# banyancomputer/hot-proofs-blake3-circom

Measured on AMD Instinct MI355X. Metric: BLAKE3-compression witnesses/sec, higher is better.
Workload: dtype u32

## Files before the change

hot-proofs-blake3-circom_amd/build.py:

```python
import os, shutil, subprocess, sys

PKG = os.path.dirname(os.path.abspath(__file__))
ROOT = os.path.dirname(PKG)
CSRC = os.path.join(PKG, "csrc")
LIB = os.path.join(PKG, "libb3wit.so")
NAPI = os.path.join(PKG, "js", "b3wit_napi.node")
ARCH = "gfx950"


def _newer(target, sources):
    if not os.path.exists(target):
        return True
    t = os.path.getmtime(target)
    return any(os.path.getmtime(s) > t for s in sources)


def _run(cmd, **kw):
    print("+", " ".join(cmd), flush=True)
    subprocess.check_call(cmd, **kw)


def hipcc():
    for c in (os.environ.get("HIPCC"), shutil.which("hipcc"), "/opt/rocm/bin/hipcc"):
        if c and os.path.exists(c):
            return c
    raise RuntimeError("hipcc not found")


def build_lib(force=False, extra_flags=()):
    from concurrent.futures import ThreadPoolExecutor
    names = ("b3w_kernels.hip", "b3w_exact.hip", "b3w_plan.hip", "b3w_bao.hip", "b3w_bao_have.hip", "b3w_bao_host.cpp", "b3w_placement.hip", "b3w_commit.hip", "b3w_r1cs.hip", "b3w_r1cs_walk.hip", "b3w_r1cs_host.cpp", "b3w_hostcomm.cpp",
             "b3w_ctx.cpp", "b3w_bodies.cpp", "b3w_wtns.cpp", "b3w_r1cs_api.cpp", "b3w_commit_api.cpp", "b3w_comm.cpp", "b3w_chain.cpp")
    srcs = [os.path.join(CSRC, f) for f in names]
    hdrs = [os.path.join(CSRC, f) for f in sorted(os.listdir(CSRC)) if f.endswith((".h", ".inc"))] + \
        [os.path.join(ROOT, "include", "b3wit.h")]
    objdir = os.path.join(PKG, "build")
    os.makedirs(objdir, exist_ok=True)
    if os.environ.get("B3W_BUILD_DIAG") == "1":
        extra_flags = (*extra_flags, "-DB3W_R1CS_DIAG")
    flags = [f"--offload-arch={ARCH}", "-O3", "-std=c++17", "-fPIC", "-x", "hip", "-Wall", "-Wno-unused-function", *extra_flags]
    jobs = []
    for src in srcs:
        obj = os.path.join(objdir, os.path.basename(src) + ".o")
        if force or extra_flags or _newer(obj, [src] + hdrs):
            jobs.append([hipcc(), *flags, "-c", src, "-o", obj])
    if jobs:
        with ThreadPoolExecutor(max_workers=min(len(jobs), os.cpu_count() or 1)) as ex:
            list(ex.map(_run, jobs))
    objs = [os.path.join(objdir, os.path.basename(src) + ".o") for src in srcs]
    if jobs or _newer(LIB, objs):
        _run([hipcc(), f"--offload-arch={ARCH}", "-fPIC", "-shared", "-o", LIB, *objs, "-ldl", "-lrt", "-lpthread"])
    return LIB


def build_oracle(force=False):
    so = os.path.join(ROOT, "oracle", "libb3w_oracle.so")
    if force or _newer(so, [os.path.join(ROOT, "oracle", "b3w_oracle.c")]):
        _run(["make", "-C", os.path.join(ROOT, "oracle")])
    return so


def build_napi(force=False):
    src = os.path.join(PKG, "js", "b3wit_napi.cc")
    if not os.path.exists(src):
        return None
    inc = "/usr/include/node"
    if not os.path.exists(os.path.join(inc, "node_api.h")):
        print("node_api.h not found; skipping N-API addon", file=sys.stderr)
        return None
    if force or _newer(NAPI, [src, os.path.join(ROOT, "include", "b3wit.h")]):
        _run(["g++", "-O2", "-std=c++17", "-fPIC", "-shared", "-DNODE_GYP_MODULE_NAME=b3wit_napi", "-I", inc,
              "-I", os.path.join(ROOT, "include"), "-o", NAPI, src, "-ldl"])
    return NAPI


def build_all(force=False):
    build_lib(force)
    build_oracle(force)
    build_napi(force)


if __name__ == "__main__":
    build_all(force="--force" in sys.argv)
```

hot-proofs-blake3-circom_amd/csrc/b3w_ctx.cpp:

```cpp
#include "b3w_internal.h"
#include "b3w_layout_tables.inc"
#include "b3w_trace_tables.inc"

namespace {

struct Sha256 {
  uint32_t h[8];
  uint8_t buf[64];
  uint64_t len = 0;
  size_t fill = 0;
  Sha256() {
    static const uint32_t init[8] = {0x6a09e667, 0xbb67ae85, 0x3c6ef372, 0xa54ff53a, 0x510e527f, 0x9b05688c, 0x1f83d9ab, 0x5be0cd19};
    memcpy(h, init, sizeof h);
  }
  static uint32_t ror(uint32_t x, int r) { return (x >> r) | (x << (32 - r)); }
  void block(const uint8_t *p) {
    static const uint32_t K[64] = {
        0x428a2f98, 0x71374491, 0xb5c0fbcf, 0xe9b5dba5, 0x3956c25b, 0x59f111f1, 0x923f82a4, 0xab1c5ed5, 0xd807aa98, 0x12835b01,
        0x243185be, 0x550c7dc3, 0x72be5d74, 0x80deb1fe, 0x9bdc06a7, 0xc19bf174, 0xe49b69c1, 0xefbe4786, 0x0fc19dc6, 0x240ca1cc,
        0x2de92c6f, 0x4a7484aa, 0x5cb0a9dc, 0x76f988da, 0x983e5152, 0xa831c66d, 0xb00327c8, 0xbf597fc7, 0xc6e00bf3, 0xd5a79147,
        0x06ca6351, 0x14292967, 0x27b70a85, 0x2e1b2138, 0x4d2c6dfc, 0x53380d13, 0x650a7354, 0x766a0abb, 0x81c2c92e, 0x92722c85,
        0xa2bfe8a1, 0xa81a664b, 0xc24b8b70, 0xc76c51a3, 0xd192e819, 0xd6990624, 0xf40e3585, 0x106aa070, 0x19a4c116, 0x1e376c08,
        0x2748774c, 0x34b0bcb5, 0x391c0cb3, 0x4ed8aa4a, 0x5b9cca4f, 0x682e6ff3, 0x748f82ee, 0x78a5636f, 0x84c87814, 0x8cc70208,
        0x90befffa, 0xa4506ceb, 0xbef9a3f7, 0xc67178f2};
    uint32_t w[64];
    for (int i = 0; i < 16; i++) w[i] = (uint32_t)p[4 * i] << 24 | (uint32_t)p[4 * i + 1] << 16 | (uint32_t)p[4 * i + 2] << 8 | p[4 * i + 3];
    for (int i = 16; i < 64; i++) {
      uint32_t s0 = ror(w[i - 15], 7) ^ ror(w[i - 15], 18) ^ (w[i - 15] >> 3);
      uint32_t s1 = ror(w[i - 2], 17) ^ ror(w[i - 2], 19) ^ (w[i - 2] >> 10);
      w[i] = w[i - 16] + s0 + w[i - 7] + s1;
    }
    uint32_t a = h[0], b = h[1], c = h[2], d = h[3], e = h[4], f = h[5], g = h[6], hh = h[7];
    for (int i = 0; i < 64; i++) {
      uint32_t t1 = hh + (ror(e, 6) ^ ror(e, 11) ^ ror(e, 25)) + ((e & f) ^ (~e & g)) + K[i] + w[i];
      uint32_t t2 = (ror(a, 2) ^ ror(a, 13) ^ ror(a, 22)) + ((a & b) ^ (a & c) ^ (b & c));
      hh = g; g = f; f = e; e = d + t1; d = c; c = b; b = a; a = t1 + t2;
    }
    h[0] += a; h[1] += b; h[2] += c; h[3] += d; h[4] += e; h[5] += f; h[6] += g; h[7] += hh;
  }
  void update(const uint8_t *p, size_t n) {
    len += n;
    while (n) {
      size_t k = 64 - fill < n ? 64 - fill : n;
      memcpy(buf + fill, p, k);
      fill += k; p += k; n -= k;
      if (fill == 64) { block(buf); fill = 0; }
    }
  }
  void final(uint8_t out[32]) {
    uint64_t bits = len * 8;
    uint8_t pad = 0x80;
    update(&pad, 1);
    uint8_t z = 0;
    while (fill != 56) update(&z, 1);
    uint8_t lb[8];
    for (int i = 0; i < 8; i++) lb[i] = (uint8_t)(bits >> (56 - 8 * i));
    update(lb, 8);
    for (int i = 0; i < 8; i++) { out[4 * i] = h[i] >> 24; out[4 * i + 1] = h[i] >> 16; out[4 * i + 2] = h[i] >> 8; out[4 * i + 3] = h[i]; }
  }
};

const char *const WASM_SHA256[4] = {
    "6faf23ddfd697bbb7e8e922577589c2c06486258968a5a14f96fb5a16091b142",
    "020bd11f289864c54c7d02cd05723dcf8323e31fa5c77d8700c618232685978e",
    "b982f960ebbfcabe957fe13857ea47adfeee30e18fbe05474e9b982eab187f46",
    "8d6317b72eab34d34e12dfd7bd310dce40f4190768669772f992a9510c441fca"};


uint64_t fnv1a64(const char *s) {
  uint64_t h = 0xCBF29CE484222325ull;
  for (; *s; ++s) { h ^= (uint8_t)*s; h *= 0x100000001B3ull; }
  return h;
}
const CircuitDesc CIRCUITS[4] = {
    {B3W_KIND_COMP, 24093, 28, 16, P_BN254, B3W_LAYOUT_0, B3W_LAYOUT_0_NRUNS, B3W_LDS_WORDS_COMP},
    {B3W_KIND_NOVA_O2, 23291, 32, 15, P_BN254, B3W_LAYOUT_1, B3W_LAYOUT_1_NRUNS, B3W_LDS_WORDS_NOVA_O2},
    {B3W_KIND_NOVA_O2, 23291, 32, 15, P_VESTA, B3W_LAYOUT_2, B3W_LAYOUT_2_NRUNS, B3W_LDS_WORDS_NOVA_O2},
    {B3W_KIND_NOVA_O1, 24614, 32, 15, P_BN254, B3W_LAYOUT_3, B3W_LAYOUT_3_NRUNS, B3W_LDS_WORDS_NOVA_O1},
};

bool atom_lds(int kind, uint32_t atom, uint32_t *word, int *width ) {
  if (atom < B3W_A_HG) { *word = atom; *width = 32; return true; }
  if (atom < B3W_A_NV) {
    const uint32_t k = (atom - B3W_A_HG) / 8, j = (atom - B3W_A_HG) % 8;
    static const uint32_t off[8] = {0, 0, 2, 2, 4, 5, 6, 7};
    *word = B3W_LDS_HG + 8 * k + off[j];
    *width = (j == B3W_HG_S1 || j == B3W_HG_S3) ? 64 : 32;
    return true;
  }
  if (kind == B3W_KIND_COMP) return false;
  const uint32_t i = atom - B3W_A_NV;
  if (i == NV_CHUNK_IDX) { *word = B3W_LDS_CHUNK_IDX; *width = 64; return true; }
  if (i < NV_NARROW_COUNT) { *word = B3W_LDS_NV + i; *width = 32; return true; }
  if (i >= NV_COUNT) return false;
  uint32_t j = i - NV_NARROW_COUNT;
  if (kind == B3W_KIND_NOVA_O2) {
    if (j < 3) {  }
    else if (i >= NV_EQ_INV && i < NV_EQ_INV + 64) j = 3 + (i - NV_EQ_INV);
    else return false;
  }
  *word = B3W_LDS_WIDE + 8 * j;
  *width = 256;
  return true;
}

void inv_small_host(uint32_t k, const uint32_t P[8], uint32_t out[8]) {
  uint64_t r = 0;
  for (int i = 7; i >= 0; --i) r = ((r << 32) | P[i]) % k;
  int64_t x0 = 0, x1 = 1;
  uint64_t a = k, b = r;
  while (b > 1) {
    const uint64_t q = a / b, tt = a - q * b;
    a = b; b = tt;
    const int64_t tx = x0 - (int64_t)q * x1;
    x0 = x1; x1 = tx;
  }
  int64_t x = x1 % (int64_t)k;
  if (x < 0) x += k;
  const uint64_t t = ((uint64_t)k - (uint64_t)x) % k;
  uint32_t prod[9];
  uint64_t carry = 1;
  for (int i = 0; i < 8; ++i) {
    const uint64_t cur = (uint64_t)P[i] * t + carry;
    prod[i] = (uint32_t)cur;
    carry = cur >> 32;
  }
  prod[8] = (uint32_t)carry;
  uint64_t rem = 0;
  for (int i = 8; i >= 0; --i) {
    const uint64_t cur = (rem << 32) | prod[i];
    const uint64_t qd = cur / k;
    rem = cur - qd * k;
    if (i < 8) out[i] = (uint32_t)qd;
  }
}
std::vector<uint32_t> build_nova_aux(const uint64_t *prime) {
  std::vector<uint32_t> aux(16 + 8 * B3W_INV_TABLE_N, 0);
  memcpy(aux.data(), prime, 32);
  aux[8] = B3W_INV_TABLE_N;
  for (uint32_t k = 1; k < B3W_INV_TABLE_N; ++k) inv_small_host(k, aux.data(), aux.data() + 16 + 8 * k);
  return aux;
}

bool build_slot_table(const CircuitDesc &c, std::vector<uint32_t> &table, std::string &err) {
  const uint32_t padded = ((c.nwit + 31) / 32 + 8) * 32;
  table.assign(padded, B3W_ENTRY(0, 31, B3W_MODE_BIT));
  std::vector<uint8_t> seen(c.nwit, 0);
  char msg[128];
  for (uint32_t r = 0; r < c.nruns; r++) {
    const b3w_layout_run &run = c.runs[r];
    for (uint32_t j = 0; j < run.len; j++) {
      const uint32_t slot = run.slot + j;
      if (slot >= c.nwit || seen[slot]) { err = "layout: bad or duplicate slot"; return false; }
      seen[slot] = 1;
      uint32_t word; int width;
      if (run.kind == 'W') {
        if (!atom_lds(c.kind, run.atom + j, &word, &width)) {
          snprintf(msg, sizeof msg, "layout: atom %u not staged for this circuit kind", run.atom + j);
          err = msg; return false;
        }
        table[slot] = B3W_ENTRY(word, 0, width == 32 ? B3W_MODE_W32 : width == 64 ? B3W_MODE_W64 : B3W_MODE_W256);
      } else {
        const uint32_t bit = run.bit0 + j;
        if (run.atom == B3W_A_NV + NV_CHUNK_IDX && bit == 64) {
          table[slot] = B3W_ENTRY(B3W_A_ONE, 31, B3W_MODE_BIT);
          continue;
        }
        if (!atom_lds(c.kind, run.atom, &word, &width) || (int)bit >= width || width == 256) {
          snprintf(msg, sizeof msg, "layout: bit %u of atom %u not expressible", bit, run.atom);
          err = msg; return false;
        }
        table[slot] = B3W_ENTRY(word + bit / 32, bit % 32, B3W_MODE_BIT);
      }
    }
  }
  for (uint32_t s = 0; s < c.nwit; s++) if (!seen[s]) { err = "layout: uncovered slot"; return false; }
  return true;
}

bool build_exact_table(const CircuitDesc &c, std::vector<uint32_t> &table) {
  table.assign(c.nwit, 0);
  for (uint32_t r = 0; r < c.nruns; r++) {
    const b3w_layout_run &run = c.runs[r];
    for (uint32_t j = 0; j < run.len; j++) {
      const uint32_t slot = run.slot + j;
      if (slot >= c.nwit) return false;
      if (run.kind == 'W') table[slot] = (run.atom + j) | (0xFFFFu << 16);
      else table[slot] = (run.atom == B3W_A_NV + NV_CIL ? B3W_A_NV + NV_CHUNK_IDX : run.atom) | ((run.bit0 + j) << 16);
    }
  }
  return true;
}

bool reference_trace(int circuit, uint32_t site, std::string &text) {
  static const b3w_trace_entry *const T[4] = {B3W_TRACES_0, B3W_TRACES_1, B3W_TRACES_2, B3W_TRACES_3};
  static const uint32_t N[4] = {B3W_TRACES_0_N, B3W_TRACES_1_N, B3W_TRACES_2_N, B3W_TRACES_3_N};
  const uint32_t code = site & 0xFF, r = (site >> 8) & 0xF;
  const bool later = code == 1 && r >= 1 && r <= 6;
  const uint32_t key = later ? site & ~0xF00u : site;
  for (uint32_t i = 0; i < N[circuit]; i++) {
    if (T[circuit][i].site != key) continue;
    text = T[circuit][i].text;
    if (!later) return true;
    const std::string frame = "Error in template Blake3Compression_";
    const size_t at = text.find(frame), num = at == std::string::npos ? at : text.find(" line: ", at), end = num == std::string::npos ? num : text.find('\n', num);
    if (end == std::string::npos) return false;
    text.replace(num + 7, end - (num + 7), circuit == 0 ? "207" : "208");
    return true;
  }
  return false;
}

bool build_input_slots(const CircuitDesc &c, std::vector<uint32_t> &slots) {
  slots.assign(c.nin, 0xFFFFFFFFu);
  const uint32_t first = c.kind == B3W_KIND_COMP ? B3W_A_H : B3W_A_NV;
  for (uint32_t r = 0; r < c.nruns; r++) {
    const b3w_layout_run &run = c.runs[r];
    if (run.kind != 'W') continue;
    for (uint32_t j = 0; j < run.len; j++) {
      const uint32_t atom = run.atom + j;
      if (atom >= first && atom < first + c.nin && slots[atom - first] == 0xFFFFFFFFu) slots[atom - first] = run.slot + j;
    }
  }
  for (uint32_t v : slots) if (v == 0xFFFFFFFFu) return false;
  return true;
}

const char *assert_site_text(uint32_t site, char *buf, size_t len) {
  const uint32_t code = site & 0xFF, r = (site >> 8) & 0xF, g = (site >> 12) & 0xF, hf = (site >> 16) & 1;
  switch (code) {
    case 1: snprintf(buf, len, "Error in template Bits34 line: 201 (rounds[%u].GS[%u].half%u.add1)\n", r, g, hf + 1); break;
    case 2: snprintf(buf, len, "Error in template ToBits line: 153 (rounds[%u].GS[%u].half%u.rxor2.tb)\n", r, g, hf + 1); break;
    case 3: snprintf(buf, len, "Error in template Bits33 line: 176 (rounds[%u].GS[%u].half%u.add3)\n", r, g, hf + 1); break;
    case 4: snprintf(buf, len, "Error in template ToBits line: 153 (rounds[%u].GS[%u].half%u.rxor4.tb)\n", r, g, hf + 1); break;
    case 5: snprintf(buf, len, "Error in template ToBits line: 153 (outXor[%u].tb_x)\n", g + 8 * hf); break;
    case 6: snprintf(buf, len, "Error in template ToBits line: 153 (outXor[%u].tb_y)\n", g + 8 * hf); break;
    case 10: snprintf(buf, len, "Error in template Num2Bits line: 38 (check_depth.check_parent.n2b)\n"); break;
    case 11: snprintf(buf, len, "Error in template Num2Bits line: 38 (check_depth.exceed_depth.lt.n2b)\n"); break;
    case 12: snprintf(buf, len, "Error in template Blake3NovaTreePath_CheckDepth line: 38\n"); break;
    case 13: snprintf(buf, len, "Error in template Num2Bits line: 38 (final_m.down_left_path.n2b)\n"); break;
    case 14: snprintf(buf, len, "Error in template Blake3GetDownLeftPath line: 77\n"); break;
    default: snprintf(buf, len, "assert site %u\n", site);
  }
  return buf;
}

}

bool b3w_int_build_slot_table(const CircuitDesc &c, std::vector<uint32_t> &table, std::string &err) { return build_slot_table(c, table, err); }

namespace {
int32_t ensure_scratch(b3w_ctx *ctx) {
  if (ctx->d_scratch) return B3W_OK;
  ctx->scratch_cap = B3W_SWEEP_CHUNK;
  hipError_t e = hipMalloc((void **)&ctx->d_scratch, (size_t)ctx->scratch_cap * ctx->desc.lds_words * 4);
  if (e != hipSuccess) { ctx->scratch_cap = 0; return hip_fail(ctx, e, "hipMalloc(sweep scratch)"); }
  return B3W_OK;
}

void set_inputs(b3w_ctx *ctx) {
  struct Def { const char *name; uint32_t count; };
  static const Def comp[] = {{"h", 8}, {"m", 16}, {"t", 2}, {"b", 1}, {"d", 1}};
  static const Def nova[] = {{"n_blocks", 1}, {"block_count", 1}, {"h", 8}, {"chunk_idx_low", 1}, {"chunk_idx_high", 1},
                             {"leaf_depth", 1}, {"total_depth", 1}, {"depth", 1}, {"m", 16}, {"b", 1}};
  const Def *d = ctx->desc.kind == B3W_KIND_COMP ? comp : nova;
  const int nd = ctx->desc.kind == B3W_KIND_COMP ? 5 : 10;
  uint32_t off = 0;
  for (int i = 0; i < nd; i++) {
    ctx->inputs.push_back({d[i].name, d[i].count, off, fnv1a64(d[i].name)});
    off += d[i].count;
  }
}
}

int b3w_int_default_variant(const b3w_ctx *ctx, uint32_t n, const uint8_t *d_bodies, uint64_t pitch) {
  const bool comp = ctx->desc.kind == B3W_KIND_COMP, nova2 = ctx->desc.kind == B3W_KIND_NOVA_O2;
  const bool fillable = ctx->fill_ok && !(reinterpret_cast<uintptr_t>(d_bodies) & 31) && !(pitch & 31) && pitch < (1ull << 30) &&
                        (uint64_t)n * pitch + (1ull << 20) < (1ull << 37);
  if (fillable && comp && n >= 128 && (n <= 3072 || !b3w_place_is_mixed(d_bodies))) return B3W_VARIANT_REGIONFILL;
  if (fillable && nova2 && (b3w_place_is_mixed(d_bodies) ? n >= 768 && n <= 2560 : n >= 512)) return B3W_VARIANT_REGIONFILL;
  if (n <= 2560) return B3W_VARIANT_SLICED + (n <= (comp ? 32u : 8u) ? 64 : n <= 96 ? 32 : n <= 192 ? 16 : n <= 768 ? 8 : 4);
  if (comp) return n <= 6144 ? 0 : 8;
  if (nova2) return n <= 3072 ? 0 : n <= 32768 ? 3 : 4;
  return 0;
}

extern "C" {

uint32_t b3w_abi_version(void) { return (1u << 16) | 4u; }

int32_t b3w_identify_wasm(const uint8_t *code, size_t len) {
  if (!code) return B3W_CIRCUIT_UNKNOWN;
  Sha256 s;
  s.update(code, len);
  uint8_t dg[32];
  s.final(dg);
  char hex[65];
  for (int i = 0; i < 32; i++) snprintf(hex + 2 * i, 3, "%02x", dg[i]);
  for (int c = 0; c < 4; c++) if (!strcmp(hex, WASM_SHA256[c])) return c;
  return B3W_CIRCUIT_UNKNOWN;
}

int32_t b3w_create(int32_t circuit, int32_t device, b3w_ctx **out) {
  if (!out || circuit < 0 || circuit > 3) return B3W_E_BAD_ARGUMENT;
  *out = nullptr;
  int ndev = 0;
  if (hipGetDeviceCount(&ndev) != hipSuccess || ndev <= 0 || device < 0 || device >= ndev) return B3W_E_NO_DEVICE;
  b3w_ctx *ctx = new b3w_ctx;
  ctx->circuit = circuit;
  ctx->desc = CIRCUITS[circuit];
  ctx->device = device;
  set_inputs(ctx);
  std::vector<uint32_t> table;
  if (!build_slot_table(ctx->desc, table, ctx->last_error)) { delete ctx; return B3W_E_BAD_ARGUMENT; }
  std::vector<uint32_t> wide_slots(B3W_NOVA_ISZERO, 0xFFFFFFFFu);
  ctx->fill_ok = ctx->desc.kind == B3W_KIND_COMP || ctx->desc.kind == B3W_KIND_NOVA_O2;
  for (uint32_t i = 0; i < table.size(); i++) {
    const uint32_t e = table[i], src = e & 0xFFFu, sh = (e >> 12) & 31u, mode = (e >> 17) & 3u;
    if (mode != B3W_MODE_BIT && sh != 0) ctx->fill_ok = false;
    if (ctx->desc.kind == B3W_KIND_COMP) {
      if (src >= 1023 || mode == B3W_MODE_W256) ctx->fill_ok = false;
    } else if (mode == B3W_MODE_W256) {
      const uint32_t j = src >= B3W_LDS_WIDE && (src - B3W_LDS_WIDE) % 8 == 0 ? (src - B3W_LDS_WIDE) / 8 : 0xFFFFFFFFu;
      if (j >= B3W_NOVA_ISZERO || wide_slots[j] != 0xFFFFFFFFu) ctx->fill_ok = false; else wide_slots[j] = i;
    } else if (src + (mode == B3W_MODE_W64 ? 1u : 0u) >= B3W_LDS_WIDE) ctx->fill_ok = false;
  }
  if (ctx->desc.kind == B3W_KIND_NOVA_O2) {
    for (uint32_t v : wide_slots) if (v == 0xFFFFFFFFu) ctx->fill_ok = false;
    for (uint32_t j = 0; ctx->fill_ok && j < B3W_NOVA_ISZERO; j++) {
      if (j > 0 && wide_slots[j] <= wide_slots[j - 1]) ctx->fill_ok = false;
      for (int d = -3; ctx->fill_ok && d <= 3; d++) {
        const int64_t k = (int64_t)wide_slots[j] + d;
        if (k < 0 || k >= (int64_t)ctx->desc.nwit) continue;
        const uint32_t e = table[k], src = e & 0xFFFu, mode = (e >> 17) & 3u;
        if (mode != B3W_MODE_W256 && !((src >= B3W_A_H && src < B3W_A_O) || src >= B3W_LDS_NV)) ctx->fill_ok = false;
      }
    }
  }
  std::vector<uint16_t> ftab(table.size(), 0);
  std::vector<uint32_t> alias;
  if (ctx->fill_ok) {
    const bool nova = ctx->desc.kind != B3W_KIND_COMP;
    std::vector<uint8_t> used(4097, 0);
    for (uint32_t i = 0; i < ctx->desc.nwit; i++) {
      const uint32_t e = table[i], src = e & 0xFFFu, mode = (e >> 17) & 3u;
      if (mode == B3W_MODE_W256) continue;
      used[src] = 1;
      if (mode == B3W_MODE_W64) used[src + 1] = 1;
    }
    used[B3W_LDS_OKWORD] = used[B3W_LDS_OKWORD + 1] = 1;
    for (uint32_t k = 0; k < 16; k++) used[B3W_A_O + k] = 1;
    if (nova) for (uint32_t k : {NV_N_BLOCKS, NV_BLOCK_COUNT_OUT, NV_TOTAL_DEPTH, NV_DEPTH_OUT, NV_CIL, NV_CIH, NV_LEAF_DEPTH}) used[B3W_LDS_NV + k] = 1;
    for (uint32_t w = 2048; w < 4097; w++) if (used[w]) ctx->fill_ok = false;
    std::vector<uint16_t> to(2048, 0xFFFFu);
    uint32_t hole = B3W_LDS_HG;
    for (uint32_t w = 1024; w < 2048 && ctx->fill_ok; w++) {
      if (!used[w]) continue;
      while (hole < 1024 && used[hole]) hole++;
      if (hole >= 1024 || alias.size() >= B3W_ALIAS_MAX) { ctx->fill_ok = false; break; }
      used[hole] = 1; to[w] = (uint16_t)hole;
      alias.push_back(w | hole << 16);
    }
    for (uint32_t i = 0; i < table.size() && ctx->fill_ok; i++) {
      const uint32_t e = table[i], sh = (e >> 12) & 31u, mode = (e >> 17) & 3u;
      uint32_t src = e & 0xFFFu;
      if (mode == B3W_MODE_W256) { ftab[i] = (uint16_t)(0x8000u | 2u << 10); continue; }
      if (src >= 1024) {
        if (mode == B3W_MODE_W64 || src >= 2048 || to[src] == 0xFFFFu) { if (i < ctx->desc.nwit) ctx->fill_ok = false; continue; }
        src = to[src];
      }
      if (mode == B3W_MODE_W64 && src + 1 >= 1024) { ctx->fill_ok = false; continue; }
      ftab[i] = (uint16_t)(mode == B3W_MODE_BIT ? (src | sh << 10) : (src | (mode == B3W_MODE_W64 ? 1u : 0u) << 10 | 0x8000u));
    }
  }
  DeviceGuard guard(device);
  if (guard.err != hipSuccess) { delete ctx; return B3W_E_NO_DEVICE; }
  const CircuitDesc &d = ctx->desc;
  hipError_t e = hipMalloc((void **)&ctx->d_table_base, (table.size() + 32) * 4 + ftab.size() * 2);
  if (e == hipSuccess) e = hipMemset(ctx->d_table_base, 0, 32 * 4);
  if (e == hipSuccess) ctx->d_table = ctx->d_table_base + 32;
  if (e == hipSuccess) e = hipMemcpy(ctx->d_table, table.data(), table.size() * 4, hipMemcpyHostToDevice);
  if (e == hipSuccess) e = hipMemcpy(ctx->d_table + table.size(), ftab.data(), ftab.size() * 2, hipMemcpyHostToDevice);
  if (e == hipSuccess && d.kind != B3W_KIND_COMP) {
    std::vector<uint32_t> aux = build_nova_aux(d.prime);
    static_assert(B3W_AUX_WIDE_SLOTS == 16 + 8 * B3W_INV_TABLE_N, "b3w_kernels.h and b3w_internal.h disagree about the inverse table");
    aux.insert(aux.end(), wide_slots.begin(), wide_slots.end());
    if (ctx->fill_ok && d.kind == B3W_KIND_NOVA_O2) {
      aux.resize(B3W_AUX_LINE_LISTS + 2 * 4 * B3W_LINE_LIST_MAX, 0xFFFFFFFFu);
      for (uint32_t ph = 0; ph < 4; ph++) {
        uint32_t cnt = 0, last_line = 0xFFFFFFFFu;
        for (uint32_t j = 0; j < B3W_NOVA_ISZERO; j++) {
          const uint32_t line = (ph + wide_slots[j]) >> 2;
          if (line == last_line) continue;
          last_line = line;
          for (uint32_t i = 0; i < 4; i++) {
            const uint32_t k = line * 4 + i - ph;
            if (k >= d.nwit) continue;
            if (cnt == B3W_LINE_LIST_MAX) { ctx->fill_ok = false; break; }
            aux[B3W_AUX_LINE_LISTS + 2 * (ph * B3W_LINE_LIST_MAX + cnt)] = k;
            aux[B3W_AUX_LINE_LISTS + 2 * (ph * B3W_LINE_LIST_MAX + cnt) + 1] = table[k];
            cnt++;
          }
        }
        aux[B3W_AUX_LINE_COUNTS + ph] = cnt;
      }
      aux.resize(B3W_AUX_ALIAS_LIST + B3W_ALIAS_MAX, 0u);
      aux[B3W_AUX_ALIAS_COUNT] = (uint32_t)alias.size();
      for (size_t k = 0; k < alias.size(); k++) aux[B3W_AUX_ALIAS_LIST + k] = alias[k];
    }
    e = hipMalloc(&ctx->d_aux, aux.size() * 4);
    if (e == hipSuccess) e = hipMemcpy(ctx->d_aux, aux.data(), aux.size() * 4, hipMemcpyHostToDevice);
  }
  {
    std::vector<uint32_t> xt;
    if (!build_exact_table(d, xt)) { b3w_destroy(ctx); return B3W_E_BAD_ARGUMENT; }
    if (e == hipSuccess) e = hipMalloc((void **)&ctx->d_exact_table, xt.size() * 4);
    if (e == hipSuccess) e = hipMemcpy(ctx->d_exact_table, xt.data(), xt.size() * 4, hipMemcpyHostToDevice);
    if (e == hipSuccess) e = hipMalloc((void **)&ctx->d_prime, 32);
    if (e == hipSuccess) e = hipMemcpy(ctx->d_prime, d.prime, 32, hipMemcpyHostToDevice);
    if (e == hipSuccess) e = hipMalloc((void **)&ctx->d_fe_inputs, 32 * 32);
    if (e == hipSuccess) e = hipMalloc((void **)&ctx->d_status2, 8);
    std::vector<uint32_t> ins;
    if (build_input_slots(d, ins)) {
      if (e == hipSuccess) e = hipMalloc((void **)&ctx->d_in_slots, ins.size() * 4);
      if (e == hipSuccess) e = hipMemcpy(ctx->d_in_slots, ins.data(), ins.size() * 4, hipMemcpyHostToDevice);
    }
  }
  if (e == hipSuccess) e = hipMalloc((void **)&ctx->d_rec1, d.nin * 4);
  if (e == hipSuccess) e = hipMalloc((void **)&ctx->d_body1, (size_t)d.nwit * 32);
  if (e == hipSuccess) e = hipMalloc((void **)&ctx->d_status1, 4);
  if (e != hipSuccess) { b3w_destroy(ctx); return B3W_E_HIP; }
  const char *v = getenv("B3W_VARIANT");
  if (v) { ctx->variant = atoi(v); ctx->variant_auto = false; }
  if (ctx->variant >= B3W_VARIANT_SWEEP && ctx->variant < B3W_VARIANT_REGIONFILL && ensure_scratch(ctx) != B3W_OK) { b3w_destroy(ctx); return B3W_E_HIP; }
  *out = ctx;
  return B3W_OK;
}

void b3w_destroy(b3w_ctx *ctx) {
  if (!ctx) return;
  B3wCaptureRelaxed relaxed;
  DeviceGuard guard(ctx->device);
  (void)b3w_ctx_trim(ctx);
  if (ctx->d_table_base) (void)hipFree(ctx->d_table_base);
  if (ctx->d_aux) (void)hipFree(ctx->d_aux);
  if (ctx->d_scratch) (void)hipFree(ctx->d_scratch);
  if (ctx->d_exact_table) (void)hipFree(ctx->d_exact_table);
  if (ctx->d_prime) (void)hipFree(ctx->d_prime);
  if (ctx->d_fe_inputs) (void)hipFree(ctx->d_fe_inputs);
  if (ctx->d_status2) (void)hipFree(ctx->d_status2);
  if (ctx->d_in_slots) (void)hipFree(ctx->d_in_slots);
  if (ctx->d_rec1) (void)hipFree(ctx->d_rec1);
  if (ctx->d_body1) (void)hipFree(ctx->d_body1);
  if (ctx->d_status1) (void)hipFree(ctx->d_status1);
  if (ctx->samples_done) { (void)hipEventSynchronize(ctx->samples_done); (void)hipEventDestroy(ctx->samples_done); }
  if (ctx->h_samples) (void)hipHostFree(ctx->h_samples);
  if (ctx->d_samples) (void)hipFree(ctx->d_samples);
  if (ctx->batch_done) { (void)hipEventSynchronize(ctx->batch_done); (void)hipEventDestroy(ctx->batch_done); }
  if (ctx->h_batch) (void)hipHostFree(ctx->h_batch);
  if (ctx->d_batch) (void)hipFree(ctx->d_batch);
  for (b3w_ctx::ManySlot &m : ctx->many_slots) {
    if (m.done) { if (m.busy) (void)hipEventSynchronize(m.done); (void)hipEventDestroy(m.done); }
    if (m.h) (void)hipHostFree(m.h);
    if (m.d) (void)hipFree(m.d);
  }
  delete ctx;
}

int32_t b3w_info(const b3w_ctx *ctx, uint32_t *n32, uint8_t prime_le[32], uint32_t *witness_size,
                 uint32_t *input_size, uint32_t version[3]) {
  if (!ctx) return B3W_E_BAD_ARGUMENT;
  if (n32) *n32 = 8;
  if (prime_le) memcpy(prime_le, ctx->desc.prime, 32);
  if (witness_size) *witness_size = ctx->desc.nwit;
  if (input_size) *input_size = ctx->desc.nin;
  if (version) { version[0] = 2; version[1] = 1; version[2] = 6; }
  return B3W_OK;
}

int32_t b3w_input_signal_size(const b3w_ctx *ctx, uint64_t h) {
  if (!ctx) return 0;
  for (const InputSignal &s : ctx->inputs) if (s.hash == h) return (int32_t)s.count;
  return 0;
}

uint32_t b3w_public_words(const b3w_ctx *ctx) { return ctx ? ctx->desc.npub : 0; }

int32_t b3w_last_error(const b3w_ctx *ctx, char *buf, size_t len) {
  if (!ctx || !buf || !len) return B3W_E_BAD_ARGUMENT;
  snprintf(buf, len, "%s", ctx->last_error.c_str());
  return B3W_OK;
}

int32_t b3w_write_wtns_header(const b3w_ctx *ctx, uint8_t out[76]) {
  if (!ctx || !out) return B3W_E_BAD_ARGUMENT;
  uint32_t w[19];
  memcpy(&w[0], "wtns", 4);
  w[1] = 2; w[2] = 2;
  w[3] = 1; w[4] = 8 + 32; w[5] = 0;
  w[6] = 32;
  memcpy(&w[7], ctx->desc.prime, 32);
  w[15] = ctx->desc.nwit;
  const uint64_t len = 32ull * ctx->desc.nwit;
  w[16] = 2; w[17] = (uint32_t)len; w[18] = (uint32_t)(len >> 32);
  memcpy(out, w, 76);
  return B3W_OK;
}

int32_t b3w_batch_run_device(b3w_ctx *ctx, const uint32_t *d_records, uint32_t n, uint8_t *d_bodies, uint64_t pitch,
                             uint32_t *d_public, int32_t *d_status, void *stream) {
  if (!ctx || !d_records || !d_bodies) return B3W_E_BAD_ARGUMENT;
  const uint64_t body = 32ull * ctx->desc.nwit;
  if (pitch == 0) pitch = body;
  if (pitch < body || (pitch & 31)) { ctx->last_error = "pitch must be >= witness_size*32 and a multiple of 32"; return B3W_E_BAD_ARGUMENT; }
  if (reinterpret_cast<uintptr_t>(d_bodies) & 15) { ctx->last_error = "d_bodies must be 16-byte aligned"; return B3W_E_BAD_ARGUMENT; }
  ON_DEVICE(ctx);
  int variant = ctx->variant;
  if (ctx->variant_auto || (ctx->variant_tuned && n <= 2560)) variant = b3w_int_default_variant(ctx, n, d_bodies, pitch);
  if (variant >= B3W_VARIANT_REGIONFILL && !ctx->fill_ok) { ctx->last_error = "the fill-ordered variants (200, 201) exist for the compression circuit and the nova O2 builds"; return B3W_E_BAD_ARGUMENT; }
  int rc = b3w_launch_batch(ctx->desc.kind, variant, d_records, n, d_bodies, pitch, ctx->d_table, ctx->desc.nwit,
                            d_public, d_status, ctx->d_aux, ctx->d_scratch, ctx->scratch_cap, (hipStream_t)stream);
  if (rc == 0) return B3W_OK;
  if (rc == -5) { ctx->last_error = "the sweep and fill-ordered paths need 32-byte aligned bodies and pitch < 2^30"; return B3W_E_BAD_ARGUMENT; }
  if (rc < 0) { ctx->last_error = "no kernel for this circuit kind / variant"; return B3W_E_BAD_ARGUMENT; }
  return hip_fail(ctx, (hipError_t)rc, "kernel launch");
}

int32_t b3w_batch_verify_device(b3w_ctx *ctx, const uint8_t *d_bodies, uint32_t n, uint64_t pitch, uint32_t *d_mismatch,
                                void *stream) {
  if (!ctx || !d_bodies || !d_mismatch) return B3W_E_BAD_ARGUMENT;
  if (!ctx->d_in_slots) { ctx->last_error = "this circuit's layout does not keep every input as a slot"; return B3W_E_BAD_ARGUMENT; }
  const uint64_t body = 32ull * ctx->desc.nwit;
  if (pitch == 0) pitch = body;
  if (pitch < body || (pitch & 31) || (reinterpret_cast<uintptr_t>(d_bodies) & 15)) {
    ctx->last_error = "pitch must be >= witness_size*32 and a multiple of 32, bodies 16-byte aligned";
    return B3W_E_BAD_ARGUMENT;
  }
  ON_DEVICE(ctx);
  int rc = b3w_launch_verify(ctx->desc.kind, ctx->d_in_slots, n, d_bodies, pitch, ctx->d_table, ctx->desc.nwit, d_mismatch,
                             ctx->d_aux, (hipStream_t)stream);
  return rc ? hip_fail(ctx, (hipError_t)rc, "verify launch") : B3W_OK;
}

int32_t b3w_batch_autotune_device(b3w_ctx *ctx, const uint32_t *d_records, uint32_t n, uint8_t *d_bodies, uint64_t pitch,
                                  uint32_t *d_public, int32_t *d_status, void *stream, int32_t *chosen_variant,
                                  float *chosen_ms) {
  if (!ctx || !d_records || !d_bodies || !n) return B3W_E_BAD_ARGUMENT;
  ON_DEVICE(ctx);
  int32_t rc;
  if (n <= 2560 && (ctx->variant_auto || ctx->variant_tuned)) {
    float ms = 0;
    rc = B3W_OK;
    for (int w = 0; w < 2 && rc == B3W_OK; w++) rc = b3w_batch_run_device(ctx, d_records, n, d_bodies, pitch, d_public, d_status, stream);
    if (rc == B3W_OK) rc = b3w_batch_time_device(ctx, d_records, n, d_bodies, pitch, d_public, d_status, stream, 5, &ms);
    if (rc) return rc;
    if (chosen_variant) *chosen_variant = b3w_int_default_variant(ctx, n, d_bodies, pitch ? pitch : 32ull * ctx->desc.nwit);
    if (chosen_ms) *chosen_ms = ms;
    return B3W_OK;
  }
  rc = ensure_scratch(ctx);
  if (rc) return rc;
  const int candidates[6] = {0, ctx->desc.kind == B3W_KIND_COMP ? (n > 6144 ? 8 : 3) : ctx->desc.kind == B3W_KIND_NOVA_O2 ? 3 : 0, B3W_VARIANT_SWEEP,
                             ctx->fill_ok ? B3W_VARIANT_REGIONFILL : 0, ctx->desc.kind == B3W_KIND_NOVA_O2 && n >= 16384 ? 4 : 0,
                             ctx->fill_ok ? B3W_VARIANT_REGIONFILL_LIGHT : 0};
  int best = ctx->variant;
  float best_ms = 1e30f;
  const int saved = ctx->variant;
  const bool saved_auto = ctx->variant_auto;
  ctx->variant_auto = false;
  float cand_ms[6] = {1e30f, 1e30f, 1e30f, 1e30f, 1e30f, 1e30f};
  for (int round = 0; round < 2; round++) {
    for (int ci = 0; ci < 6; ci++) {
      const int c = candidates[ci];
      if (ci > 0 && c == candidates[0]) continue;
      if (round > 0 && cand_ms[ci] >= 1e30f) continue;
      ctx->variant = c;
      float ms = 0;
      rc = B3W_OK;
      for (int w = 0; w < 2 && rc == B3W_OK; w++)
        rc = b3w_batch_run_device(ctx, d_records, n, d_bodies, pitch, d_public, d_status, stream);
      if (rc == B3W_OK) rc = b3w_batch_time_device(ctx, d_records, n, d_bodies, pitch, d_public, d_status, stream, n <= 8192 ? 20 : 5, &ms);
      if (rc == B3W_E_BAD_ARGUMENT) continue;
      if (rc) { ctx->variant = saved; ctx->variant_auto = saved_auto; return rc; }
      if (ms < cand_ms[ci]) cand_ms[ci] = ms;
    }
  }
  for (int ci = 0; ci < 6; ci++)
    if (cand_ms[ci] < best_ms) { best_ms = cand_ms[ci]; best = candidates[ci]; }
  if (best_ms >= 1e30f) { ctx->variant = saved; ctx->variant_auto = saved_auto; return B3W_E_BAD_ARGUMENT; }
  ctx->variant = best;
  ctx->variant_tuned = true;
  if (chosen_variant) *chosen_variant = best;
  if (chosen_ms) *chosen_ms = best_ms;
  return B3W_OK;
}

int32_t b3w_batch_time_device(b3w_ctx *ctx, const uint32_t *d_records, uint32_t n, uint8_t *d_bodies, uint64_t pitch,
                              uint32_t *d_public, int32_t *d_status, void *stream, uint32_t iters, float *avg_ms) {
  if (!ctx || !avg_ms || !iters) return B3W_E_BAD_ARGUMENT;
  ON_DEVICE(ctx);
  hipEvent_t e0 = nullptr, e1 = nullptr;
  hipError_t e = hipEventCreate(&e0);
  if (e == hipSuccess) e = hipEventCreate(&e1);
  if (e == hipSuccess) e = hipEventRecord(e0, (hipStream_t)stream);
  int32_t rc = B3W_OK;
  for (uint32_t i = 0; i < iters && e == hipSuccess && rc == B3W_OK; i++)
    rc = b3w_batch_run_device(ctx, d_records, n, d_bodies, pitch, d_public, d_status, stream);
  float ms = 0;
  if (e == hipSuccess && rc == B3W_OK) e = hipEventRecord(e1, (hipStream_t)stream);
  if (e == hipSuccess && rc == B3W_OK) e = hipEventSynchronize(e1);
  if (e == hipSuccess && rc == B3W_OK) e = hipEventElapsedTime(&ms, e0, e1);
  if (e0) (void)hipEventDestroy(e0);
  if (e1) (void)hipEventDestroy(e1);
  if (rc) return rc;
  if (e != hipSuccess) return hip_fail(ctx, e, "timing events");
  *avg_ms = ms / iters;
  return B3W_OK;
}

static int32_t calc_witness_run(b3w_ctx *ctx, const std::vector<uint32_t> &rec, const std::vector<uint8_t> &fe, bool canonical,
                                uint8_t *out_body) {
  const CircuitDesc &d = ctx->desc;
  char msg[200];
  ON_DEVICE(ctx);
  if (canonical) {
    HIP_TRY(ctx, hipMemcpy(ctx->d_rec1, rec.data(), d.nin * 4, hipMemcpyHostToDevice));
    int32_t rc = b3w_batch_run_device(ctx, ctx->d_rec1, 1, ctx->d_body1, 0, nullptr, ctx->d_status1, nullptr);
    if (rc) return rc;
    int32_t st = 0;
    HIP_TRY(ctx, hipMemcpy(&st, ctx->d_status1, 4, hipMemcpyDeviceToHost));
    if (st == 0) {
      HIP_TRY(ctx, hipMemcpy(out_body, ctx->d_body1, (size_t)d.nwit * 32, hipMemcpyDeviceToHost));
      return B3W_OK;
    }
  }
  HIP_TRY(ctx, hipMemcpy(ctx->d_fe_inputs, fe.data(), fe.size(), hipMemcpyHostToDevice));
  int rc = b3w_launch_exact(d.kind != B3W_KIND_COMP, ctx->d_fe_inputs, ctx->d_prime, ctx->d_exact_table, d.nwit,
                            ctx->d_body1, ctx->d_status2, nullptr);
  if (rc) return hip_fail(ctx, (hipError_t)rc, "exact kernel launch");
  uint32_t st2[2] = {0, 0};
  HIP_TRY(ctx, hipMemcpy(st2, ctx->d_status2, 8, hipMemcpyDeviceToHost));
  if (st2[0] != 0) {
    if (!reference_trace(ctx->circuit, st2[1], ctx->last_error))
      ctx->last_error = std::string("Assert Failed.\n") + assert_site_text(st2[1], msg, sizeof msg);
    return B3W_E_ASSERT_FAILED;
  }
  HIP_TRY(ctx, hipMemcpy(out_body, ctx->d_body1, (size_t)d.nwit * 32, hipMemcpyDeviceToHost));
  return B3W_OK;
}

int32_t b3w_calc_witness(b3w_ctx *ctx, const uint64_t *name_hashes, const uint32_t *counts, const uint8_t *values_le32,
                         uint32_t nkeys, uint8_t *out_body) {
  if (!ctx || !name_hashes || !counts || !values_le32 || !out_body) return B3W_E_BAD_ARGUMENT;
  const CircuitDesc &d = ctx->desc;
  std::vector<uint32_t> rec(d.nin, 0);
  std::vector<uint8_t> fe((size_t)d.nin * 32, 0);
  std::vector<uint8_t> set(d.nin, 0);
  uint32_t nset = 0;
  bool canonical = true, ran = false;
  const uint8_t *v = values_le32;
  char msg[200];
  for (uint32_t k = 0; k < nkeys; k++) {
    const InputSignal *sig = nullptr;
    for (const InputSignal &s : ctx->inputs) if (s.hash == name_hashes[k]) sig = &s;
    const uint32_t size = sig ? sig->count : 0;
    if (counts[k] < size) { ctx->last_error = std::string("Not enough values for input signal ") + (sig ? sig->name : "?") + "\n"; return B3W_E_ARRAY_ACCESS; }
    if (counts[k] > size) { ctx->last_error = std::string("Too many values for input signal ") + (sig ? sig->name : "?") + "\n"; return B3W_E_TOO_MANY_SIGNALS; }
    for (uint32_t i = 0; i < size; i++, v += 32) {
      const uint32_t idx = sig->rec_off + i;
      if (set[idx]) { ctx->last_error = "Signal already set.\n"; return B3W_E_SIGNAL_ALREADY_SET; }
      memcpy(&fe[(size_t)idx * 32], v, 32);
      memcpy(&rec[idx], v, 4);
      for (int b = 4; b < 32; b++) canonical &= (v[b] == 0);
      set[idx] = 1;
      nset++;
    }
    if (!ran && size > 0 && nset == d.nin) {
      const int32_t rc = calc_witness_run(ctx, rec, fe, canonical, out_body);
      if (rc) return rc;
      ran = true;
    }
  }
  if (nset < d.nin) {
    snprintf(msg, sizeof msg, "Not all inputs have been set. Only %u out of %u", nset, d.nin);
    ctx->last_error = msg;
    return B3W_E_NOT_ALL_INPUTS;
  }
  return B3W_OK;
}

}
```

hot-proofs-blake3-circom_amd/csrc/b3w_internal.h:

```cpp
#pragma once
#include <hip/hip_runtime_api.h>
#include <hip/hip_ext.h>
#include <errno.h>
#include <fcntl.h>
#include <stdint.h>
#include <stdio.h>
#include <stdlib.h>
#include <string.h>
#include <sys/uio.h>
#include <unistd.h>
#include <algorithm>
#include <array>
#include <chrono>
#include <atomic>
#include <map>
#include <mutex>
#include <thread>
#include <string>
#include <vector>

#include "../../include/b3wit.h"
#include "b3w_atoms.h"
#include "b3w_capture.h"
#include "b3w_kernels.h"
#include "b3w_r1cs_host.h"


struct b3w_layout_run { char kind; uint32_t slot, atom, bit0, len; };

struct InputSignal { const char *name; uint32_t count; uint32_t rec_off; uint64_t hash; };

struct CircuitDesc {
  int kind;
  uint32_t nwit, nin, npub;
  const uint64_t *prime;
  const b3w_layout_run *runs;
  uint32_t nruns;
  uint32_t lds_words;
};
inline constexpr uint64_t P_BN254[4] = {0x43e1f593f0000001ull, 0x2833e84879b97091ull, 0xb85045b68181585dull, 0x30644e72e131a029ull};
inline constexpr uint64_t P_VESTA[4] = {0x8c46eb2100000001ull, 0x224698fc0994a8ddull, 0x0ull, 0x4000000000000000ull};
constexpr uint32_t B3W_INV_TABLE_N = 2048;

struct b3w_ctx {
  int circuit = -1;
  CircuitDesc desc{};
  int device = -1;
  int variant = 0;
  bool variant_auto = true;
  bool fill_ok = false;
  bool variant_tuned = false;
  std::vector<InputSignal> inputs;
  uint32_t *d_table = nullptr;
  uint32_t *d_table_base = nullptr;
  void *d_aux = nullptr;
  uint32_t *d_scratch = nullptr;
  uint32_t *d_exact_table = nullptr;
  uint32_t *d_prime = nullptr;
  uint32_t *d_fe_inputs = nullptr;
  uint32_t *d_status2 = nullptr;
  uint32_t *d_in_slots = nullptr;
  uint32_t scratch_cap = 0;
  uint32_t *d_rec1 = nullptr;
  uint8_t *d_body1 = nullptr;
  int32_t *d_status1 = nullptr;
  float plain_ms_per_gb = 0;
  struct Spare { void *ptr; uint64_t bytes; int32_t placement; };
  std::vector<Spare> ring_spares;
  uint64_t *h_samples = nullptr, *d_samples = nullptr;
  uint32_t samples_cap = 0;
  hipEvent_t samples_done = nullptr;
  uint8_t *h_batch = nullptr, *d_batch = nullptr;
  uint64_t batch_cap = 0;
  hipEvent_t batch_done = nullptr;
  static constexpr uint32_t B3W_MANY_SLOTS = 8;
  struct ManySlot { uint8_t *h = nullptr, *d = nullptr; uint64_t cap = 0; hipEvent_t done = nullptr; bool busy = false; };
  ManySlot many_slots[B3W_MANY_SLOTS];
  uint32_t many_next = 0;
  std::string last_error;
};

struct b3w_batch {
  b3w_ctx *ctx = nullptr;
  uint32_t capacity = 0, n = 0;
  uint64_t pitch = 0;
  int32_t placement = B3W_PLACEMENT_PLAIN;
  uint32_t *d_recs = nullptr;
  uint8_t *d_bodies = nullptr;
  uint32_t *d_pub = nullptr;
  int32_t *d_status = nullptr;
};

inline int32_t hip_fail(b3w_ctx *ctx, hipError_t e, const char *what) {
  if (ctx) ctx->last_error = std::string(what) + ": " + hipGetErrorString(e);
  return B3W_E_HIP;
}
inline int32_t refuse(b3w_ctx *ctx, const char *call, const std::string &why) {
  ctx->last_error = call ? std::string(call) + ": " + why : why;
  return B3W_E_BAD_ARGUMENT;
}
inline int32_t group_log_ok(b3w_ctx *ctx, const char *call, uint32_t group_log) {
  return group_log > B3W_BAO_MAX_GROUP_LOG ? refuse(ctx, call, "group_log is above B3W_BAO_MAX_GROUP_LOG (6)") : B3W_OK;
}
#define HIP_TRY(ctx, call)                                  \
  do {                                                      \
    hipError_t _e = (call);                                 \
    if (_e != hipSuccess) return hip_fail(ctx, _e, #call);  \
  } while (0)

#define B3W_TRY(...)                  \
  do {                                \
    const int32_t _rc = (__VA_ARGS__);\
    if (_rc) return _rc;              \
  } while (0)

struct DeviceGuard {
  int prev = -1;
  bool switched = false;
  hipError_t err = hipSuccess;
  explicit DeviceGuard(int dev) {
    err = hipGetDevice(&prev);
    if (err == hipSuccess && prev != dev) {
      err = hipSetDevice(dev);
      switched = err == hipSuccess;
    }
  }
  ~DeviceGuard() { if (switched) (void)hipSetDevice(prev); }
  DeviceGuard(const DeviceGuard &) = delete;
  DeviceGuard &operator=(const DeviceGuard &) = delete;
};
#define ON_DEVICE(ctx)                         \
  DeviceGuard _dev_guard((ctx)->device);       \
  if (_dev_guard.err != hipSuccess) return hip_fail(ctx, _dev_guard.err, "hipSetDevice")

bool b3w_int_build_slot_table(const CircuitDesc &c, std::vector<uint32_t> &table, std::string &err);
int b3w_int_default_variant(const b3w_ctx *ctx, uint32_t n, const uint8_t *d_bodies, uint64_t pitch);
b3w_ctx *b3w_int_key_ctx(const b3w_commit_key *key);
int32_t b3w_int_commit_records(b3w_ctx *ctx, const b3w_commit_key *key, const uint32_t *d_records, uint32_t n, uint8_t *d_points, uint32_t *d_public,
                               int32_t *d_status, void *stream, uint32_t *d_sums_out, void *trace_stream = nullptr, hipEvent_t trace_done = nullptr);
int32_t b3w_int_commit_normalize(b3w_ctx *ctx, const b3w_commit_key *key, const uint32_t *d_sums, uint64_t n, uint8_t *d_points, void *stream);
b3w_ctx *b3w_int_r1cs_ctx(const b3w_r1cs *r1cs);
int32_t b3w_int_batch_staging(b3w_ctx *ctx, uint64_t bytes);
int32_t b3w_int_batch_launched(b3w_ctx *ctx, hipStream_t st, const char *what);
constexpr uint64_t B3W_RING_SPARE_CAP = 26ull << 30;
```

hot-proofs-blake3-circom_amd/csrc/b3w_kernels.h:

```cpp
#pragma once
#include <hip/hip_runtime_api.h>
#include <stdint.h>

#define B3W_VARIANT_SWEEP 100
#define B3W_VARIANT_SLICED 20
#define B3W_VARIANT_REGIONFILL 200
#define B3W_VARIANT_REGIONFILL_LIGHT 201
#define B3W_REGIONFILL_GRID 256
#define B3W_AUX_WIDE_SLOTS (16 + 8 * 2048)
#define B3W_AUX_LINE_COUNTS (B3W_AUX_WIDE_SLOTS + 68)
#define B3W_AUX_LINE_LISTS (B3W_AUX_LINE_COUNTS + 4)
#define B3W_LINE_LIST_MAX 160
#define B3W_AUX_ALIAS_COUNT (B3W_AUX_LINE_LISTS + 2 * 4 * B3W_LINE_LIST_MAX)
#define B3W_AUX_ALIAS_LIST (B3W_AUX_ALIAS_COUNT + 1)
#define B3W_ALIAS_MAX 192
#define B3W_SWEEP_GRID 256
#define B3W_SWEEP_LOGC 13
#define B3W_SWEEP_CHUNK (1u << B3W_SWEEP_LOGC)

extern "C" int b3w_launch_batch(int kind, int variant, const uint32_t *d_recs, uint32_t n, uint8_t *d_out,
                                uint64_t pitch, const uint32_t *d_table, uint32_t nwit, uint32_t *d_pub,
                                int32_t *d_status, const void *d_aux, uint32_t *d_scratch, uint32_t scratch_cap,
                                hipStream_t stream);

extern "C" int b3w_launch_exact(int nova, const uint32_t *d_inputs, const uint32_t *d_prime, const uint32_t *d_table,
                                uint32_t nwit, uint8_t *d_out, uint32_t *d_status, hipStream_t stream);

extern "C" uint32_t b3w_plan_path_len(uint64_t chunk, uint64_t nchunks);
extern "C" int b3w_launch_plan_leaves(const uint8_t *d_pre, uint64_t total_len, uint64_t first_chunk, uint32_t nlocal,
                                      uint64_t nchunks, uint32_t *d_recs, uint32_t *d_chunk_cv, hipStream_t stream);
extern "C" int b3w_launch_plan_merge(const uint32_t *d_left, const uint32_t *d_right, uint32_t stride_words, uint64_t npairs,
                                     uint32_t root, uint32_t *d_parents, hipStream_t stream);
extern "C" int b3w_launch_plan_parents(const uint32_t *d_levels, uint64_t nchunks, uint64_t first_chunk, uint32_t nlocal,
                                       uint32_t last_chunk_blocks, uint32_t *d_recs, hipStream_t stream);
extern "C" uint32_t b3w_plan_tree_first_level(uint64_t nchunks);
extern "C" int b3w_launch_plan_tree(uint32_t *d_levels, uint64_t nchunks, uint32_t l0, uint32_t *d_root, uint64_t first_chunk, uint32_t plan_nlocal,
                                    uint32_t last_chunk_blocks, uint32_t *d_recs, hipStream_t stream);
extern "C" uint64_t b3w_plan_parent_row(uint64_t chunk, uint64_t nchunks);
extern "C" int b3w_plan_path_provable(uint64_t chunk, uint64_t nchunks);
extern "C" int b3w_launch_pack_hout(const uint32_t *d_pub, uint64_t row0, uint64_t count, uint32_t *d_dst, hipStream_t stream);
extern "C" int b3w_launch_unpack_hout(const uint32_t *d_gathered, uint64_t block_words, uint64_t par_off, const uint64_t *d_tab, uint32_t nranks,
                                      uint64_t max_rows, uint32_t *d_leaf_all, uint32_t *d_par_all, hipStream_t stream);

extern "C" int b3w_launch_trace(int kind, const uint32_t *d_recs, uint32_t cn, uint32_t *d_images, uint32_t row, const uint32_t *d_table,
                                uint32_t nwit, uint32_t *d_pub, int32_t *d_status, const void *d_aux, hipStream_t stream);
extern "C" int b3w_launch_verify(int kind, const uint32_t *d_in_slots, uint32_t n, const uint8_t *d_bodies, uint64_t pitch,
                                 const uint32_t *d_table, uint32_t nwit, uint32_t *d_mismatch, const void *d_aux,
                                 hipStream_t stream);

extern "C" int b3w_place_alloc(int device, uint64_t bytes, int want_mixed, void **out, int *mixed, float *rates);
extern "C" int b3w_place_free(void *ptr);
extern "C" int b3w_place_is_mixed(const void *ptr);
extern "C" void b3w_place_trim(void);
extern "C" void b3w_place_configure(int64_t search_gib, int64_t pool_gib);
extern "C" void b3w_place_stats(int device, uint64_t out[6]);
extern "C" void b3w_place_search_limit(double seconds);
extern "C" void b3w_place_search_stats(int device, double out[4]);
extern "C" void b3w_place_cost_breakdown(int device, double out[4]);
extern "C" int b3w_place_store_rate(uint8_t *buf, uint64_t pitch, uint32_t n, uint32_t body_bytes, int shape, uint32_t iters, hipStream_t stream, double *gbs);

#define B3W_COMMIT_WINDOW_SMALL 12
#define B3W_COMMIT_WINDOW_LARGE 16
#define B3W_COMMIT_WINDOW_XL 18
#define B3W_COMMIT_WINDOW_OK(w) ((w) == B3W_COMMIT_WINDOW_SMALL || (w) == B3W_COMMIT_WINDOW_LARGE || (w) == B3W_COMMIT_WINDOW_XL)
#define B3W_COMMIT_ENTRIES(W) ((1u << (W)) - 1u)
#define B3W_COMMIT_SUM_WORDS 36
#include "b3w_commit_curve.h"
extern "C" int b3w_launch_commit_setup(const uint32_t *d_gens, const uint32_t *d_first_v, const uint32_t *d_nbits, uint32_t nslots,
                                       uint32_t *d_points, const B3wCurve *curve, hipStream_t stream);
extern "C" int b3w_launch_commit_windows(const uint32_t *d_points, uint32_t nwin, uint32_t window, uint32_t *d_table, const B3wCurve *curve, hipStream_t stream);
extern "C" int b3w_launch_commit(const uint8_t *d_bodies, uint32_t n, uint64_t pitch, uint32_t first_slot, uint32_t nslots,
                                 const uint32_t *d_slotdesc ,
                                 const uint32_t *d_images ,
                                 uint32_t img_row, const uint32_t *d_runs , uint32_t nruns,
                                 const uint32_t *d_table, uint32_t nwin, uint32_t window, uint32_t *d_sums, uint8_t *d_out,
                                 int32_t *d_status, const uint32_t *d_invtab , uint32_t inv_nk,
                                 const uint32_t *d_invmeta ,
                                 const uint32_t *d_aux ,
                                 unsigned long long *d_adds ,
                                 const B3wCurve *curve, hipStream_t stream);
extern "C" int b3w_launch_commit_normalize(const uint32_t *d_sums, uint64_t n, uint8_t *d_out, const B3wCurve *curve, hipStream_t stream);
#define B3W_NOVA_ISZERO 67
extern "C" int b3w_launch_commit_invtab(const uint32_t *d_gens, const uint32_t *d_inv_slot, const uint32_t *d_inverses, uint32_t njobs, uint32_t nk,
                                        uint32_t *d_invtab, const B3wCurve *curve, hipStream_t stream);

#include "b3w_r1cs_defs.h"
extern "C" int b3w_launch_r1cs(const uint8_t *d_bodies, uint32_t n, uint64_t pitch, uint32_t m, const uint32_t *d_rows,
                               const uint32_t *d_row_id, const uint32_t *d_wires, const uint16_t *d_cids, const uint32_t *d_coefR,
                               const B3wField *field, uint32_t *d_violations, uint32_t *d_first, hipStream_t stream);
struct B3wR1csSystem {
  uint32_t nwires, ntiles, max_ext, max_tile_terms, max_tile_rows, ncoef;
  const uint32_t *tiles, *tile_terms, *ext, *rows, *row_id, *row_k, *terms, *coefs;
  const long long *coef_small;
  const uint32_t *g_rows, *g_wires;
  const uint16_t *g_cids;
  uint32_t max_g_words, max_g_rows, smask_groups;
  const uint32_t *srows, *sgdesc, *sgwords, *sgmeta;
  const unsigned long long *smask;
  const unsigned long long *scost;
};
struct B3wWalk {
  uint32_t ntiles, exp_slots, max_gen, max_ent, ncoef, static_words, max_rows, signed_elems;
  const uint32_t *tile;
  const unsigned long long *mask;
  const uint16_t *exp;
  const uint4 *runs;
  const uint32_t *run_row, *ent_w, *ent_m, *row_id;
  const unsigned long long *stat;
  const long long *coef_small;
  const uint32_t *static_k, *static_id;
  uint32_t nstatic, pad2;
  uint32_t static_d0[4];
  uint32_t p[8];
};
extern "C" int b3w_launch_r1cs_walk(const uint8_t *d_bodies, uint32_t n, uint64_t pitch, const B3wWalk *walk, const B3wR1csSystem *sysw, const B3wField *field,
                                    unsigned long long *d_scratch, uint32_t *d_violations, uint32_t *d_first, hipStream_t stream);
extern "C" size_t b3w_r1cs_walk_scratch_bytes(const B3wWalk *walk);
#define B3W_R1CS_SLAB 8192u
extern "C" size_t b3w_r1cs_scratch_bytes(const B3wR1csSystem *sys);
extern "C" int b3w_launch_r1cs_stream(const uint8_t *d_bodies, uint32_t n, uint64_t pitch, const B3wR1csSystem *sys, const B3wField *field,
                                      unsigned long long *d_scratch, uint32_t *d_violations, uint32_t *d_first, hipStream_t stream);
```

hot-proofs-blake3-circom_amd/csrc/b3w_kernels.hip:

```cpp
#include <hip/hip_runtime.h>
#include <stdint.h>
#include <stdlib.h>
#include <atomic>
#include "b3w_atoms.h"
#include "b3w_kernels.h"

namespace {

typedef uint32_t u32x4 __attribute__((ext_vector_type(4)));

__device__ __forceinline__ uint32_t rotr32(uint32_t x, int r) { return __builtin_rotateright32(x, r); }

template <int P0, int P1, int P2, int P3>
__device__ __forceinline__ uint32_t quad_perm(uint32_t x) {
  return (uint32_t)__builtin_amdgcn_update_dpp(0, (int)x, P0 | (P1 << 2) | (P2 << 4) | (P3 << 6), 0xF, 0xF, false);
}

__host__ __device__ constexpr uint64_t sched_pack(int r) {
  const int sigma[16] = {2, 6, 3, 10, 7, 0, 4, 13, 1, 11, 12, 5, 9, 14, 15, 8};
  int p[16] = {0, 1, 2, 3, 4, 5, 6, 7, 8, 9, 10, 11, 12, 13, 14, 15};
  for (int i = 0; i < r; i++) {
    int q[16] = {};
    for (int j = 0; j < 16; j++) q[j] = p[sigma[j]];
    for (int j = 0; j < 16; j++) p[j] = q[j];
  }
  uint64_t v = 0;
  for (int j = 0; j < 16; j++) v |= (uint64_t)p[j] << (4 * j);
  return v;
}

template <int R1, int R2>
__device__ __forceinline__ void half_g(uint32_t &a, uint32_t &b, uint32_t &c, uint32_t &d, uint32_t m,
                                       uint32_t *Lk) {
  const uint64_t s1 = (uint64_t)a + b + m;
  const uint32_t A = (uint32_t)s1;
  const uint32_t D2 = rotr32(d ^ A, R1);
  const uint64_t s3 = (uint64_t)c + D2;
  const uint32_t C = (uint32_t)s3;
  const uint32_t B4 = rotr32(b ^ C, R2);
  *reinterpret_cast<uint4 *>(Lk) = make_uint4(A, (uint32_t)(s1 >> 32), C, (uint32_t)(s3 >> 32));
  *reinterpret_cast<uint4 *>(Lk + 4) = make_uint4(D2, d, B4, b);
  a = A; d = D2; c = C; b = B4;
}

template <int R>
__device__ __forceinline__ void round_fn(uint32_t &a, uint32_t &b, uint32_t &c, uint32_t &d, const uint32_t *L,
                                         uint32_t *Lw, int col) {
  constexpr uint64_t P = sched_pack(R);
  const uint32_t *M = L + B3W_A_M;
  {
    const uint32_t mx = M[(P >> (8 * col)) & 15], my = M[(P >> (8 * col + 4)) & 15];
    uint32_t *Lk = Lw + B3W_LDS_HG + 8 * ((R * 8 + col) * 2);
    half_g<16, 12>(a, b, c, d, mx, Lk);
    half_g<8, 7>(a, b, c, d, my, Lk + 8);
  }
  b = quad_perm<1, 2, 3, 0>(b);
  c = quad_perm<2, 3, 0, 1>(c);
  d = quad_perm<3, 0, 1, 2>(d);
  {
    const uint32_t mx = M[(P >> (32 + 8 * col)) & 15], my = M[(P >> (36 + 8 * col)) & 15];
    uint32_t *Lk = Lw + B3W_LDS_HG + 8 * ((R * 8 + 4 + col) * 2);
    half_g<16, 12>(a, b, c, d, mx, Lk);
    half_g<8, 7>(a, b, c, d, my, Lk + 8);
  }
  b = quad_perm<3, 0, 1, 2>(b);
  c = quad_perm<2, 3, 0, 1>(c);
  d = quad_perm<1, 2, 3, 0>(d);
}

__device__ __forceinline__ void trace_compression(uint32_t *L, int col, uint32_t *pub ) {
  const uint32_t IVc = col == 0 ? 0x6A09E667u : col == 1 ? 0xBB67AE85u : col == 2 ? 0x3C6EF372u : 0xA54FF53Au;
  uint32_t a = L[B3W_A_H + col], b = L[B3W_A_H + 4 + col], c = IVc, d = L[B3W_A_T + col];
  const uint32_t h_lo = a, h_hi = b;
  round_fn<0>(a, b, c, d, L, L, col);
  round_fn<1>(a, b, c, d, L, L, col);
  round_fn<2>(a, b, c, d, L, L, col);
  round_fn<3>(a, b, c, d, L, L, col);
  round_fn<4>(a, b, c, d, L, L, col);
  round_fn<5>(a, b, c, d, L, L, col);
  round_fn<6>(a, b, c, d, L, L, col);
  const uint32_t o0 = a ^ c, o1 = b ^ d, o2 = c ^ h_lo, o3 = d ^ h_hi;
  L[B3W_A_O + col] = o0;
  L[B3W_A_O + 4 + col] = o1;
  L[B3W_A_O + 8 + col] = o2;
  L[B3W_A_O + 12 + col] = o3;
  if (col == 0) L[B3W_A_ONE] = 1u;
  if (pub) { pub[col] = o0; pub[4 + col] = o1; pub[8 + col] = o2; pub[12 + col] = o3; }
}

template <bool NT>
__device__ __forceinline__ void store16(uint8_t *p, uint4 v) {
  const u32x4 x = {v.x, v.y, v.z, v.w};
  if (NT) __builtin_nontemporal_store(x, reinterpret_cast<u32x4 *>(p));
  else *reinterpret_cast<u32x4 *>(p) = x;
}

template <int W, int WORDS, bool WIDE, bool NT, bool FULL>
__device__ __forceinline__ void emit_group(const uint32_t *lds, uint32_t e, uint8_t *__restrict__ out,
                                           const uint64_t (&woff)[W], uint32_t byte_off, bool in, uint32_t nact,
                                           const uint32_t *okmask) {
  const uint32_t par = threadIdx.x & 1;
  const uint32_t src = e & 0xFFFu, sh = (e >> 12) & 31u, mode = (e >> 17) & 3u;
  const uint32_t off = (WIDE && mode == B3W_MODE_W256) ? src + 4u * par : src;
  const bool live = (par == 0) || (WIDE && mode == B3W_MODE_W256);
  const uint32_t m0 = live ? (mode == B3W_MODE_BIT ? 1u : 0xFFFFFFFFu) : 0u;
  const uint32_t m1 = (live && mode >= B3W_MODE_W64) ? 0xFFFFFFFFu : 0u;
  const uint32_t m23 = (WIDE && mode == B3W_MODE_W256) ? 0xFFFFFFFFu : 0u;
#pragma unroll
  for (int w = 0; w < W; ++w) {
    if (FULL || ((uint32_t)w < nact && (!okmask || okmask[w]))) {
      const uint32_t *L = lds + w * WORDS + off;
      uint4 v;
      v.x = (L[0] >> sh) & m0;
      v.y = L[1] & m1;
      if (WIDE) { v.z = L[2] & m23; v.w = L[3] & m23; } else { v.z = 0; v.w = 0; }
      if (FULL || in) store16<NT>(out + woff[w] + byte_off, v);
    }
  }
}

struct WaveBodies {
  uint32_t first, stride;
  __device__ __forceinline__ uint32_t operator()(int w) const { return first + (uint32_t)w * stride; }
};
template <int W>
__device__ __forceinline__ WaveBodies wave_bodies(uint32_t bid, uint32_t stride) {
  return WaveBodies{(bid / stride) * (stride * W) + bid % stride, stride};
}
template <int W>
__device__ __forceinline__ uint32_t wave_active(const WaveBodies &wb, uint32_t n) {
  uint32_t a = 0;
#pragma unroll
  for (int w = 0; w < W; ++w) a += wb(w) < n ? 1u : 0u;
  return a;
}

template <int W, int WORDS, bool WIDE, bool NT>
__device__ __forceinline__ void expand(const uint32_t *lds, const uint32_t *__restrict__ table, uint32_t nwit,
                                       uint8_t *__restrict__ out, uint64_t pitch, const WaveBodies wb, uint32_t n,
                                       const uint32_t *okmask , bool all_ok,
                                       uint32_t slice = 0, uint32_t slices = 1 ) {
  constexpr int U = 4;
  const int lane = threadIdx.x;
  const uint32_t nact = wave_active<W>(wb, n);
  const uint64_t start = reinterpret_cast<uint64_t>(out) + (uint64_t)wb.first * pitch;
  const uint32_t j = (start & 31) ? 0u : (uint32_t)(start >> 5) & 3u;
  const uint32_t ntiles = (nwit + j + 31) >> 5;
  const uint32_t kf0 = j ? 1u : 0u, kf1 = (nwit + j) >> 5;
  uint64_t woff[W];
#pragma unroll
  for (int w = 0; w < W; ++w) woff[w] = (uint64_t)wb(w) * pitch + (uint32_t)lane * 16u - 32u * j;
  const uint32_t *tp = table + (lane >> 1) - j;
  uint32_t k = 0, kend_all = ntiles;
  if (slices > 1) {
    const uint32_t per = ((ntiles + slices - 1) / slices + (U - 1)) & ~(uint32_t)(U - 1);
    k = slice * per < ntiles ? slice * per : ntiles;
    kend_all = k + per < ntiles ? k + per : ntiles;
#pragma unroll
    for (int w = 0; w < W; ++w) woff[w] += (uint64_t)k * 1024u;
  }
  const uint32_t kf1s = kf1 < kend_all ? kf1 : kend_all;
  auto ragged = [&](uint32_t kend) {
    for (; k < kend; ++k) {
      const uint32_t slot = k * 32 + (lane >> 1) - j;
      emit_group<W, WORDS, WIDE, NT, false>(lds, tp[k * 32], out, woff, 0, slot < nwit, nact, okmask);
#pragma unroll
      for (int w = 0; w < W; ++w) woff[w] += 1024u;
    }
  };
  if (nact == (uint32_t)W && all_ok) {
    ragged(kf0 < kend_all ? kf0 : kend_all);
    uint32_t cur[U], nxt[U];
#pragma unroll
    for (int u = 0; u < U; ++u) cur[u] = tp[(k + u) * 32];
    for (; k + U <= kf1s; k += U) {
#pragma unroll
      for (int u = 0; u < U; ++u) nxt[u] = tp[(k + U + u) * 32];
#pragma unroll
      for (int u = 0; u < U; ++u) emit_group<W, WORDS, WIDE, NT, true>(lds, cur[u], out, woff, u * 1024u, true, nact, nullptr);
#pragma unroll
      for (int w = 0; w < W; ++w) woff[w] += U * 1024u;
#pragma unroll
      for (int u = 0; u < U; ++u) cur[u] = nxt[u];
    }
  }
  ragged(kend_all);
}

template <int W, int WORDS, bool WIDE>
__device__ __forceinline__ void expand_verify(const uint32_t *lds, const uint32_t *__restrict__ table, uint32_t nwit,
                                              const uint8_t *__restrict__ bodies, uint64_t pitch, const WaveBodies wb, uint32_t n,
                                              uint32_t (&cnt)[W]) {
  constexpr int U = 4;
  const int lane = threadIdx.x;
  const uint32_t par = lane & 1;
  const uint32_t nact = wave_active<W>(wb, n);
  const uint64_t start = reinterpret_cast<uint64_t>(bodies) + (uint64_t)wb.first * pitch;
  const uint32_t j = (start & 31) ? 0u : (uint32_t)(start >> 5) & 3u;
  const uint32_t ntiles = (nwit + j + 31) >> 5;
#pragma unroll
  for (int w = 0; w < W; ++w) cnt[w] = 0;
  for (uint32_t k0 = 0; k0 < ntiles; k0 += U) {
    uint32_t e[U];
    u32x4 got[U][W];
#pragma unroll
    for (int u = 0; u < U; ++u) {
      const uint32_t k = k0 + u < ntiles ? k0 + u : ntiles - 1;
      const int32_t slot = (int32_t)(k * 32 + (lane >> 1)) - (int32_t)j;
      const uint32_t sl = slot < 0 ? 0u : (uint32_t)slot < nwit ? (uint32_t)slot : nwit - 1;
      e[u] = table[sl];
#pragma unroll
      for (int w = 0; w < W; ++w) {
        const uint32_t body = wb((uint32_t)w < nact ? w : 0);
        got[u][w] = *reinterpret_cast<const u32x4 *>(bodies + (uint64_t)body * pitch + (uint64_t)sl * 32 + par * 16);
      }
    }
#pragma unroll
    for (int u = 0; u < U; ++u) {
      const int32_t slot = (int32_t)((k0 + u) * 32 + (lane >> 1)) - (int32_t)j;
      const bool in = k0 + u < ntiles && slot >= 0 && (uint32_t)slot < nwit;
      const uint32_t src = e[u] & 0xFFFu, sh = (e[u] >> 12) & 31u, mode = (e[u] >> 17) & 3u;
      const uint32_t off = (WIDE && mode == B3W_MODE_W256) ? src + 4u * par : src;
      const bool live = (par == 0) || (WIDE && mode == B3W_MODE_W256);
      const uint32_t m0 = live ? (mode == B3W_MODE_BIT ? 1u : 0xFFFFFFFFu) : 0u;
      const uint32_t m1 = (live && mode >= B3W_MODE_W64) ? 0xFFFFFFFFu : 0u;
      const uint32_t m23 = (WIDE && mode == B3W_MODE_W256) ? 0xFFFFFFFFu : 0u;
#pragma unroll
      for (int w = 0; w < W; ++w) {
        const uint32_t *L = lds + w * WORDS + off;
        const uint32_t x = (L[0] >> sh) & m0, y = L[1] & m1;
        const uint32_t z = WIDE ? (L[2] & m23) : 0u, t = WIDE ? (L[3] & m23) : 0u;
        const bool bad = ((got[u][w].x ^ x) | (got[u][w].y ^ y) | (got[u][w].z ^ z) | (got[u][w].w ^ t)) != 0;
        cnt[w] += (in && (uint32_t)w < nact && bad) ? 1u : 0u;
      }
    }
  }
}

__device__ __forceinline__ uint32_t body_input_word(const uint8_t *body, uint32_t slot, uint32_t &nc) {
  const uint4 *p = reinterpret_cast<const uint4 *>(body + (uint64_t)slot * 32);
  const uint4 lo = p[0], hi = p[1];
  if (lo.y | lo.z | lo.w | hi.x | hi.y | hi.z | hi.w) nc = 1;
  return lo.x;
}

template <int W>
__device__ __forceinline__ void publish_counts(uint32_t (&cnt)[W], uint32_t *__restrict__ mismatch, const WaveBodies wb, uint32_t n,
                                               const uint32_t *flags ) {
#pragma unroll
  for (int w = 0; w < W; ++w) {
    uint32_t c = cnt[w];
#pragma unroll
    for (int o = 32; o > 0; o >>= 1) c += __shfl_xor(c, o);
    if (threadIdx.x == 0 && wb(w) < n) mismatch[wb(w)] = flags[w] ? 0xFFFFFFFFu : c;
  }
}


template <int W, int WORDS>
__device__ __forceinline__ void dump_images(uint32_t *lds, uint32_t *__restrict__ scratch, uint32_t C, uint32_t wit0,
                                            uint32_t n, const uint32_t *okf) {
  const int lane = threadIdx.x;
  if (lane < W) lds[lane * WORDS + B3W_LDS_OKWORD] = okf ? okf[lane] : 1u;
  __syncthreads();
  constexpr int ROWS = 64 / W;
  const int w = lane % W, jr = lane / W;
  if (wit0 + w < n) {
#pragma unroll 4
    for (int j = jr; j < WORDS; j += ROWS) scratch[(uint64_t)j * C + wit0 + w] = lds[w * WORDS + j];
  }
}

struct SweepPos {
  uint32_t t;
  int32_t rem;
  uint32_t w_lo;
};

__device__ __forceinline__ uint32_t uni(uint32_t x) { return (uint32_t)__builtin_amdgcn_readfirstlane((int)x); }

template <int K, int NW>
struct SweepRegs {
  uint32_t e[K]; uint32_t a[K][NW]; uint32_t ok[K];
  uint32_t t[K], wlo[K]; int32_t rem[K];
  bool fast;
};

template <bool WIDE, int K, int LOGC, int PAIRS, bool SPLIT>
__global__ __launch_bounds__(128 * PAIRS, 1) void b3w_sweep_kernel(const uint32_t *__restrict__ scr, uint32_t n,
                                                                   uint8_t *__restrict__ out_base, uint32_t lead, uint32_t pitch,
                                                                   const uint32_t *__restrict__ table, uint32_t nwit) {
  constexpr int NW = WIDE ? 8 : 2;
  extern __shared__ __attribute__((aligned(16))) uint32_t tab[];
  for (uint32_t i = threadIdx.x; i < nwit; i += 128 * PAIRS) tab[i] = table[i];
  const uint32_t tid = threadIdx.x % 128u, tid32 = tid * 32u, pair = uni(threadIdx.x / 128u);
  const uint32_t G = SPLIT ? gridDim.x : gridDim.x * PAIRS;
  const uint32_t body = 32u * nwit;
  const uint64_t total = (uint64_t)lead + (uint64_t)n * pitch;
  const uint32_t ntiles_all = (uint32_t)((total + 4095) >> 12);
  const uint32_t G0 = gridDim.x;
  const uint32_t nseq = ntiles_all > blockIdx.x ? (ntiles_all - blockIdx.x + G0 - 1) / G0 : 0;
  const uint32_t share = (nseq + PAIRS - 1) / PAIRS;
  const uint32_t first_seq = SPLIT ? pair * share : pair;
  const uint32_t end_seq = SPLIT ? (first_seq + share < nseq ? first_seq + share : nseq) : nseq;
  const uint32_t ntiles = uni(end_seq > 0 ? blockIdx.x + (end_seq - 1) * G0 + 1 : 0);
  const uint64_t stride = (uint64_t)G * 4096;
  const uint32_t dq = (uint32_t)(stride / pitch), dr = (uint32_t)(stride % pitch);
  uint32_t pt = uni(blockIdx.x + G0 * first_seq), pw;
  int32_t prem;
  {
    const int64_t pos = (int64_t)((uint64_t)pt * 4096) - (int64_t)lead;
    if (pos < 0) { pw = 0; prem = (int32_t)pos; }
    else { pw = uni((uint32_t)((uint64_t)pos / pitch)); prem = (int32_t)uni((uint32_t)((uint64_t)pos % pitch)); }
  }
  __syncthreads();
  auto locate = [&](uint32_t t, int32_t rem, uint32_t w_lo, uint32_t &w, uint32_t &r32) {
    int32_t r = rem + (int32_t)tid32;
    w = w_lo;
    if (r >= (int32_t)pitch) { r -= (int32_t)pitch; w++; }
    r32 = (uint32_t)r;
    return t < ntiles && r32 < body && w < n;
  };
  auto do_table = [&](SweepRegs<K, NW> &rg) {
    bool fast = true;
#pragma unroll
    for (int k = 0; k < K; ++k) {
      rg.t[k] = pt; rg.rem[k] = prem; rg.wlo[k] = pw;
      fast = fast && pt < ntiles && prem >= 0 && (uint32_t)prem + 4096u <= body && pw < n;
      const int32_t r = prem + (int32_t)dr;
      const bool c = r >= (int32_t)pitch;
      pt = uni(pt + G);
      pw = uni(pw + dq + (c ? 1u : 0u));
      prem = (int32_t)uni((uint32_t)(c ? r - (int32_t)pitch : r));
    }
    rg.fast = fast;
#pragma unroll
    for (int k = 0; k < K; ++k) {
      if (fast) {
        rg.e[k] = (tab + ((uint32_t)rg.rem[k] >> 5))[tid];
      } else {
        uint32_t w, r32;
        const bool in = locate(rg.t[k], rg.rem[k], rg.wlo[k], w, r32);
        rg.e[k] = tab[in ? (r32 >> 5) : 0u];
      }
    }
  };
  auto do_words = [&](SweepRegs<K, NW> &rg) {
#pragma unroll
    for (int k = 0; k < K; ++k) {
      uint32_t w = rg.wlo[k];
      if (!rg.fast) {
        uint32_t r32;
        const bool in = locate(rg.t[k], rg.rem[k], rg.wlo[k], w, r32);
        w = in ? w : 0u;
      }
      const uint32_t e = rg.e[k];
      const uint32_t row = (e & 0xFFFu) << LOGC, mode = (e >> 17) & 3u;
      const uint32_t *col = scr + w;
      rg.a[k][0] = col[row];
      if (__builtin_amdgcn_ballot_w64(mode >= B3W_MODE_W64)) {
#pragma unroll
        for (int x = 1; x < NW; ++x) rg.a[k][x] = col[row + ((uint32_t)x << LOGC)];
      } else {
#pragma unroll
        for (int x = 1; x < NW; ++x) rg.a[k][x] = 0;
      }
      rg.ok[k] = WIDE ? col[(uint32_t)B3W_LDS_OKWORD << LOGC] : 1u;
    }
  };
  auto do_emit = [&](const SweepRegs<K, NW> &rg) {
#pragma unroll
    for (int k = 0; k < K; ++k) {
      const uint32_t e = rg.e[k];
      const uint32_t sh = (e >> 12) & 31u, mode = (e >> 17) & 3u;
      const uint32_t m0 = mode == B3W_MODE_BIT ? 1u : 0xFFFFFFFFu;
      const uint32_t m1 = mode >= B3W_MODE_W64 ? 0xFFFFFFFFu : 0u;
      uint4 lo, hi;
      lo.x = (rg.a[k][0] >> sh) & m0;
      lo.y = rg.a[k][1] & m1;
      if constexpr (WIDE) {
        const uint32_t m2 = mode == B3W_MODE_W256 ? 0xFFFFFFFFu : 0u;
        lo.z = rg.a[k][2] & m2; lo.w = rg.a[k][3] & m2;
        hi = make_uint4(rg.a[k][4] & m2, rg.a[k][5] & m2, rg.a[k][6] & m2, rg.a[k][7] & m2);
      } else {
        lo.z = 0; lo.w = 0;
        hi = make_uint4(0, 0, 0, 0);
      }
      bool in = true;
      if (!rg.fast) { uint32_t w, r32; in = locate(rg.t[k], rg.rem[k], rg.wlo[k], w, r32); }
      uint8_t *dst = out_base + (uint64_t)rg.t[k] * 4096;
      if (in && (!WIDE || rg.ok[k] != 0)) {
        store16<false>(dst + tid32, lo);
        store16<false>(dst + tid32 + 16, hi);
      }
    }
  };

  SweepRegs<K, NW> r0, r1, r2;
  do_table(r0);
  do_table(r1);
  do_words(r0);
  while (true) {
    if (r0.t[0] >= ntiles) break;
    do_table(r2); do_words(r1); do_emit(r0);
    if (r1.t[0] >= ntiles) break;
    do_table(r0); do_words(r2); do_emit(r1);
    if (r2.t[0] >= ntiles) break;
    do_table(r1); do_words(r0); do_emit(r2);
  }
}

template <int W, bool NT, int MODE, bool SL = false, bool PERSIST = false>
__global__ __launch_bounds__(64) void b3w_compression_kernel(const uint32_t *__restrict__ recs, uint32_t n,
                                                             uint8_t *__restrict__ out, uint64_t pitch,
                                                             const uint32_t *__restrict__ table, uint32_t nwit,
                                                             uint32_t *__restrict__ pub, int32_t *__restrict__ status,
                                                             uint32_t stride , uint32_t slices = 1) {
  constexpr int WORDS = B3W_LDS_WORDS_COMP;
  __shared__ __attribute__((aligned(16))) uint32_t lds[W * WORDS + 4];
  const int lane = threadIdx.x;
  const uint32_t slice = SL ? blockIdx.x % slices : 0u;
  if (SL && slice != 0) { pub = nullptr; status = nullptr; }
 for (uint32_t bid = blockIdx.x;; bid += gridDim.x) {
  const WaveBodies wb = wave_bodies<W>(SL ? bid / slices : bid, stride);
  if (wb.first >= n) return;
  const uint32_t wit0 = wb.first;
  __shared__ uint32_t ncf[W];
  if (lane < W) ncf[lane] = 0;
  if (MODE == 2) __syncthreads();
  for (int i = lane; i < W * 28; i += 64) {
    const int w = i / 28, j = i - w * 28;
    if (wb(w) < n) {
      uint32_t v;
      if (MODE == 2) {
        uint32_t nc = 0;
        v = body_input_word(out + (uint64_t)wb(w) * pitch, recs[j], nc);
        if (nc) ncf[w] = 1;
      } else {
        v = recs[(uint64_t)wb(w) * 28 + j];
      }
      lds[w * WORDS + B3W_A_H + j] = v;
    }
  }
  __syncthreads();
  {
    const int w = lane >> 2, col = lane & 3;
    if (w < W && wb(w) < n) {
      trace_compression(lds + w * WORDS, col, (MODE != 2 && pub) ? pub + (uint64_t)wb(w) * 16 : nullptr);
      if (MODE != 2 && status && col == 0) status[wb(w)] = 0;
    }
  }
  __syncthreads();
  if (MODE == 1) dump_images<W, WORDS>(lds, reinterpret_cast<uint32_t *>(out), (uint32_t)pitch, wit0, n, nullptr);
  else if (MODE == 2) {
    uint32_t cnt[W];
    expand_verify<W, WORDS, false>(lds, table, nwit, out, pitch, wb, n, cnt);
    publish_counts<W>(cnt, pub, wb, n, ncf);
  } else if (SL) expand<W, WORDS, false, NT>(lds, table, nwit, out, pitch, wb, n, nullptr, true, slice, slices);
  else expand<W, WORDS, false, NT>(lds, table, nwit, out, pitch, wb, n, nullptr, true);
  if (!PERSIST) return;
  __syncthreads();
 }
}



#define B3W_AUX_TABLE 16

struct U256 { uint32_t l[8]; };

__device__ __forceinline__ U256 u256_sub(const U256 &a, const U256 &b) {
  U256 r;
  uint32_t br = 0;
#pragma unroll
  for (int i = 0; i < 8; ++i) {
    const uint64_t d = (uint64_t)a.l[i] - b.l[i] - br;
    r.l[i] = (uint32_t)d;
    br = (uint32_t)(d >> 63);
  }
  return r;
}

__device__ __forceinline__ U256 u256_small(uint64_t x) {
  U256 r;
  r.l[0] = (uint32_t)x; r.l[1] = (uint32_t)(x >> 32);
#pragma unroll
  for (int i = 2; i < 8; ++i) r.l[i] = 0;
  return r;
}

__device__ __forceinline__ U256 u256_signed(int64_t k, const U256 &P) {
  return k >= 0 ? u256_small((uint64_t)k) : u256_sub(P, u256_small((uint64_t)(-k)));
}

__device__ __forceinline__ U256 inv_small_general(uint32_t k, const U256 &P) {
  uint64_t r = 0;
#pragma unroll
  for (int i = 7; i >= 0; --i) r = ((r << 32) | P.l[i]) % k;
  int64_t x0 = 0, x1 = 1;
  uint64_t a = k, b = r;
  while (b > 1) {
    const uint64_t q = a / b, tt = a - q * b;
    a = b; b = tt;
    const int64_t tx = x0 - (int64_t)q * x1;
    x0 = x1; x1 = tx;
  }
  int64_t x = x1 % (int64_t)k;
  if (x < 0) x += k;
  const uint64_t t = ((uint64_t)k - (uint64_t)x) % k;
  uint32_t prod[9];
  uint64_t carry = 1;
#pragma unroll
  for (int i = 0; i < 8; ++i) {
    const uint64_t cur = (uint64_t)P.l[i] * t + carry;
    prod[i] = (uint32_t)cur;
    carry = cur >> 32;
  }
  prod[8] = (uint32_t)carry;
  U256 out;
  uint64_t rem = 0;
#pragma unroll
  for (int i = 8; i >= 0; --i) {
    const uint64_t cur = (rem << 32) | prod[i];
    const uint64_t qd = cur / k;
    rem = cur - qd * k;
    if (i < 8) out.l[i] = (uint32_t)qd;
  }
  return out;
}

__device__ __forceinline__ bool inv_signed(int64_t k, const U256 &P, const uint32_t *__restrict__ aux, U256 &out) {
  const uint64_t mag = k < 0 ? (uint64_t)(-k) : (uint64_t)k;
  if (mag == 0) { out = u256_small(0); return true; }
  if (mag >> 32) { out = u256_small(0); return false; }
  const uint32_t tn = aux[8];
  U256 v;
  if (mag < tn) {
    const uint4 *tp = reinterpret_cast<const uint4 *>(aux + B3W_AUX_TABLE + 8 * mag);
    const uint4 lo = tp[0], hi = tp[1];
    v.l[0] = lo.x; v.l[1] = lo.y; v.l[2] = lo.z; v.l[3] = lo.w;
    v.l[4] = hi.x; v.l[5] = hi.y; v.l[6] = hi.z; v.l[7] = hi.w;
  } else {
    v = inv_small_general((uint32_t)mag, P);
  }
  out = k < 0 ? u256_sub(P, v) : v;
  return true;
}

__device__ __forceinline__ void lds_put256(uint32_t *L, const U256 &v) {
  *reinterpret_cast<uint4 *>(L) = make_uint4(v.l[0], v.l[1], v.l[2], v.l[3]);
  *reinterpret_cast<uint4 *>(L + 4) = make_uint4(v.l[4], v.l[5], v.l[6], v.l[7]);
}

template <bool O1, bool INV>
__device__ __forceinline__ bool nova_iszero_job(uint32_t *L, int j, const U256 &P, const uint32_t *__restrict__ aux) {
  const uint32_t *in = L + B3W_LDS_NV;
  const int64_t depth = in[NV_DEPTH];
  int64_t k, in1 = 0;
  uint32_t flag_atom, isz_wide = 0, in1_wide = 0;
  if (j == 0) { k = -depth; flag_atom = NV_IS_ROOT; isz_wide = NV_ROOT_ISZ_IN; }
  else if (j == 1) { k = -(int64_t)in[NV_BLOCK_COUNT]; flag_atom = NV_E0; isz_wide = NV_E0_ISZ_IN; }
  else if (j == 2) { in1 = (int64_t)in[NV_N_BLOCKS] - 1; k = in1 - (int64_t)in[NV_BLOCK_COUNT];
                     flag_atom = NV_E1; isz_wide = NV_E1_ISZ_IN; in1_wide = NV_E1_IN1; }
  else { const int i = j - 3; in1 = (int64_t)in[NV_TOTAL_DEPTH] - i - 2; k = in1 - depth;
         flag_atom = NV_EQ_OUT + i; isz_wide = NV_EQ_ISZ_IN + i; in1_wide = NV_EQ_IN1 + i; }
  L[B3W_LDS_NV + flag_atom] = (k == 0) ? 1u : 0u;
  if (!INV) return ((uint64_t)(k < 0 ? -k : k) >> 32) == 0;
  U256 inv;
  const bool ok = inv_signed(k, P, aux, inv);
  if (!O1) {
    lds_put256(L + B3W_LDS_WIDE + 8 * j, inv);
  } else {
    const uint32_t inv_wide = j < 3 ? (uint32_t)j : (uint32_t)(NV_EQ_INV - NV_NARROW_COUNT + (j - 3));
    lds_put256(L + B3W_LDS_WIDE + 8 * inv_wide, inv);
    lds_put256(L + B3W_LDS_WIDE + 8 * (isz_wide - NV_NARROW_COUNT), u256_signed(k, P));
    if (in1_wide) lds_put256(L + B3W_LDS_WIDE + 8 * (in1_wide - NV_NARROW_COUNT), u256_signed(in1, P));
  }
  return ok;
}

__device__ __forceinline__ bool nova_iszero_flags_quad(uint32_t *L, int col) {
  uint32_t *nv = L + B3W_LDS_NV;
  const int64_t depth = nv[NV_DEPTH], block_count = nv[NV_BLOCK_COUNT], n_blocks = nv[NV_N_BLOCKS], total_depth = nv[NV_TOTAL_DEPTH];
  if (col == 0) {
    nv[NV_IS_ROOT] = depth == 0 ? 1u : 0u;
    nv[NV_E0] = block_count == 0 ? 1u : 0u;
    nv[NV_E1] = n_blocks - 1 - block_count == 0 ? 1u : 0u;
  }
  const int64_t istar = total_depth - 2 - depth;
#pragma unroll
  for (int q = 0; q < 16; ++q) {
    const int i = col * 16 + q;
    nv[NV_EQ_OUT + i] = istar == i ? 1u : 0u;
  }
  const int64_t k2 = n_blocks - 1 - block_count;
  const int64_t mag2 = k2 < 0 ? -k2 : k2, magl = istar < 0 ? -istar : istar, magh = istar - 63 < 0 ? 63 - istar : istar - 63;
  return (mag2 >> 32) != 0 || (magl >> 32) != 0 || (magh >> 32) != 0;
}

__device__ __forceinline__ int32_t nova_select(uint32_t *L, int col, bool dom_a ) {
  uint32_t *nv = L + B3W_LDS_NV;
  const uint32_t n_blocks = nv[NV_N_BLOCKS], block_count = nv[NV_BLOCK_COUNT], cil = nv[NV_CIL], cih = nv[NV_CIH];
  const uint32_t leaf_depth = nv[NV_LEAF_DEPTH], total_depth = nv[NV_TOTAL_DEPTH], depth = nv[NV_DEPTH];
  const int64_t cp = (int64_t)depth + 257 - (int64_t)leaf_depth;
  const int64_t ed = (int64_t)leaf_depth + 255 - (int64_t)depth;
  const bool assert_fail = cp < 0 || cp >= 512 || ed < 0 || ed >= 512 || ((ed >> 8) & 1) == 0;
  const uint32_t parent = 1u - (uint32_t)((cp >> 8) & 1);
  const uint32_t is_root = depth == 0 ? 1u : 0u;
  const uint32_t e0 = block_count == 0 ? 1u : 0u;
  const uint32_t e1 = ((int64_t)n_blocks - 1 == (int64_t)block_count) ? 1u : 0u;
  const bool dom = dom_a || depth == 0xFFFFFFFFu || (block_count == 0xFFFFFFFFu && !parent);
  const int32_t st = assert_fail ? 4 : dom ? 103 : 0;
  const uint32_t last = e1 & (1u - parent), first = e0 & (1u - parent);
  const uint32_t ur_tmp = parent | e1, ur_flag = ur_tmp & is_root;
  const uint32_t dflag = first + 2u * last + 8u * ur_flag + 4u * parent;
  const int64_t istar = (int64_t)total_depth - 2 - (int64_t)depth;
  const uint64_t chunk_idx = (uint64_t)cil | ((uint64_t)cih << 32);
  const bool has_star = istar >= 0 && istar < 64;
  const uint32_t nb_star = has_star ? 1u - (uint32_t)((chunk_idx >> (istar & 63)) & 1) : 0u;
  const uint32_t dl = parent ? nb_star : 1u;
  const uint32_t cdd = last | parent, decr = cdd & (1u - is_root);
  if (col == 0) {
    nv[NV_BLOCK_COUNT_OUT] = block_count + (1u - parent);
    nv[NV_DEPTH_OUT] = depth - decr;
    nv[NV_IS_PARENT] = parent;
    nv[NV_CP_IN1] = leaf_depth - 1u;
    nv[NV_CP_N2B_IN] = (uint32_t)cp;
    nv[NV_ED_IN1] = depth + 1u;
    nv[NV_ED_N2B_IN] = (uint32_t)ed;
    nv[NV_ED_OUT] = 0u;
    nv[NV_NOT_ROOT] = 1u - is_root;
    nv[NV_NOT_PARENT] = 1u - parent;
    nv[NV_IS_LAST_BLOCK] = last;
    nv[NV_FIRST] = first;
    nv[NV_UR_TMP] = ur_tmp;
    nv[NV_UR_FLAG] = ur_flag;
    nv[NV_DL] = dl;
    nv[NV_CDD_OUT] = cdd;
    nv[NV_DECR_DEPTH] = decr;
    L[B3W_LDS_CHUNK_IDX] = cil;
    L[B3W_LDS_CHUNK_IDX + 1] = cih;
    L[B3W_A_T] = parent ? 0u : cil;
    L[B3W_A_T + 1] = parent ? 0u : cih;
    L[B3W_A_B] = nv[NV_B];
    L[B3W_A_D] = dflag;
  }
#pragma unroll
  for (int q = 0; q < 4; ++q) {
    const int i = col + 4 * q;
    const uint32_t hsel = nv[NV_H + (i & 7)], msel = nv[NV_M + (i & 7)], mi = nv[NV_M + i];
    const uint32_t take_h = i < 8 ? dl : 1u - dl;
    const uint32_t td = take_h ? hsel : 0u;
    const uint32_t mp = (take_h ? 0u : msel) + td;
    const uint32_t tp = parent ? mp : 0u;
    nv[NV_TMP_DOWN + i] = td;
    nv[NV_M_IS_PARENT + i] = mp;
    nv[NV_TMP_IS_PAR + i] = tp;
    L[B3W_A_M + i] = (parent ? 0u : mi) + tp;
  }
#pragma unroll
  for (int q = 0; q < 2; ++q) {
    const int i = col + 4 * q;
    const uint32_t iv = i == 0 ? 0x6A09E667u : i == 1 ? 0xBB67AE85u : i == 2 ? 0x3C6EF372u : i == 3 ? 0xA54FF53Au
                      : i == 4 ? 0x510E527Fu : i == 5 ? 0x9B05688Cu : i == 6 ? 0x1F83D9ABu : 0x5BE0CD19u;
    const uint32_t tiv = parent ? iv : 0u;
    nv[NV_TMPIV + i] = tiv;
    L[B3W_A_H + i] = (parent ? 0u : nv[NV_H + i]) + tiv;
  }
#pragma unroll
  for (int q = 0; q < 16; ++q) {
    const int i = col * 16 + q;
    nv[NV_BIT_AT_DEPTH + i] = (has_star && (int64_t)i >= istar) ? nb_star : 0u;
  }
  return st;
}

template <int KIND, int W, bool NT, int MODE, bool SL = false, bool PERSIST = false>
__global__ __launch_bounds__(64) void b3w_nova_kernel(const uint32_t *__restrict__ recs, uint32_t n,
                                                      uint8_t *__restrict__ out, uint64_t pitch,
                                                      const uint32_t *__restrict__ table, uint32_t nwit,
                                                      uint32_t *__restrict__ pub, int32_t *__restrict__ status,
                                                      const uint32_t *__restrict__ aux, uint32_t stride, uint32_t slices = 1) {
  constexpr bool O1 = KIND == B3W_KIND_NOVA_O1;
  constexpr int WORDS = O1 ? B3W_LDS_WORDS_NOVA_O1 : B3W_LDS_WORDS_NOVA_O2;
  __shared__ __attribute__((aligned(16))) uint32_t lds[W * WORDS + 4];
  __shared__ uint32_t okf[W];
  __shared__ uint32_t domf[W];
  const int lane = threadIdx.x;
  const uint32_t slice = SL ? blockIdx.x % slices : 0u;
  if (SL && slice != 0) { pub = nullptr; status = nullptr; }
  __shared__ uint32_t ncf[W];
  U256 P;
#pragma unroll
  for (int i = 0; i < 8; ++i) P.l[i] = aux[i];
 for (uint32_t bid = blockIdx.x;; bid += gridDim.x) {
  const WaveBodies wb = wave_bodies<W>(SL ? bid / slices : bid, stride);
  if (wb.first >= n) return;
  const uint32_t wit0 = wb.first;
  if (lane < W) { okf[lane] = 0; domf[lane] = 0; ncf[lane] = 0; }
  if (MODE == 2) __syncthreads();
  for (int i = lane; i < W * 32; i += 64) {
    const int w = i >> 5, j = i & 31;
    if (wb(w) < n) {
      uint32_t v;
      if (MODE == 2) {
        uint32_t nc = 0;
        v = body_input_word(out + (uint64_t)wb(w) * pitch, recs[j], nc);
        if (nc) ncf[w] = 1;
      } else {
        v = recs[(uint64_t)wb(w) * 32 + j];
      }
      lds[w * WORDS + B3W_LDS_NV + j] = v;
    }
  }
  __syncthreads();

  for (int t = lane; t < 67 * W; t += 64) {
    const int w = t / 67, j = t - w * 67;
    if (wb(w) >= n) continue;
    if (!nova_iszero_job<O1, true>(lds + w * WORDS, j, P, aux)) domf[w] = 1;
  }
  __syncthreads();

  const int w = lane >> 2, col = lane & 3;
  const bool active = w < W && wb(w) < n;
  uint32_t *L = lds + (active ? w : 0) * WORDS;
  if (active) {
    const int32_t st = nova_select(L, col, domf[w] != 0);
    if (col == 0) {
      okf[w] = st == 0 ? 1u : 0u;
      if (MODE != 2 && status) status[wb(w)] = st;
    }
  }
  __syncthreads();
  if (MODE == 3) {
    const uint2 *lists = reinterpret_cast<const uint2 *>(aux + B3W_AUX_LINE_LISTS);
    const uint32_t half = (uint32_t)lane & 1u;
#pragma unroll
    for (int ww = 0; ww < W; ++ww) {
      if (wb(ww) < n && okf[ww]) {
        uint8_t *base = out + (uint64_t)wb(ww) * pitch;
        const uint32_t ph = (uint32_t)(reinterpret_cast<uint64_t>(base) >> 5) & 3u;
        const uint32_t cnt = aux[B3W_AUX_LINE_COUNTS + ph];
        constexpr int IT = B3W_LINE_LIST_MAX / 32;
        uint2 it[IT];
#pragma unroll
        for (int u = 0; u < IT; ++u) {
          const uint32_t idx = ((uint32_t)lane >> 1) + 32u * u;
          it[u] = idx < cnt ? lists[ph * B3W_LINE_LIST_MAX + idx] : make_uint2(0xFFFFFFFFu, 0u);
        }
#pragma unroll
        for (int u = 0; u < IT; ++u) {
          if (it[u].x < nwit) {
            const uint32_t e = it[u].y, src = e & 0xFFFu, sh = (e >> 12) & 31u, mode = (e >> 17) & 3u;
            const uint32_t *L = lds + ww * WORDS + src + (mode == B3W_MODE_W256 ? 4u * half : 0u);
            uint4 v = make_uint4(0, 0, 0, 0);
            if (mode == B3W_MODE_W256) v = make_uint4(L[0], L[1], L[2], L[3]);
            else if (!half) { v.x = mode == B3W_MODE_BIT ? (L[0] >> sh) & 1u : L[0]; v.y = mode == B3W_MODE_W64 ? L[1] : 0u; }
            store16<false>(base + (uint64_t)it[u].x * 32 + 16 * half, v);
          }
        }
      }
    }
    if (!PERSIST) return;
    __syncthreads();
    continue;
  }
  if (active && okf[w]) trace_compression(L, col, nullptr);
  __syncthreads();
  bool all_ok = true;
#pragma unroll
  for (int x = 0; x < W; ++x) all_ok = all_ok && (okf[x] != 0);
  if (MODE != 2 && active && okf[w] && pub) {
    uint32_t *pw = pub + (uint64_t)wb(w) * 15;
    const uint32_t *nv = L + B3W_LDS_NV;
    if (col == 0) { pw[0] = nv[NV_N_BLOCKS]; pw[1] = nv[NV_BLOCK_COUNT_OUT]; pw[10] = nv[NV_TOTAL_DEPTH]; pw[11] = nv[NV_DEPTH_OUT]; }
    if (col == 1) { pw[12] = nv[NV_CIL]; pw[13] = nv[NV_CIH]; pw[14] = nv[NV_LEAF_DEPTH]; }
    pw[2 + col] = L[B3W_A_O + col];
    pw[6 + col] = L[B3W_A_O + 4 + col];
  }
  if (MODE == 1) dump_images<W, WORDS>(lds, reinterpret_cast<uint32_t *>(out), (uint32_t)pitch, wit0, n, okf);
  else if (MODE == 2) {
    if (lane < W) ncf[lane] |= okf[lane] ? 0u : 1u;
    __syncthreads();
    uint32_t cnt[W];
    expand_verify<W, WORDS, true>(lds, table, nwit, out, pitch, wb, n, cnt);
    publish_counts<W>(cnt, pub, wb, n, ncf);
  } else if (SL) expand<W, WORDS, true, NT>(lds, table, nwit, out, pitch, wb, n, okf, all_ok, slice, slices);
  else expand<W, WORDS, true, NT>(lds, table, nwit, out, pitch, wb, n, okf, all_ok);
  if (!PERSIST) return;
  __syncthreads();
 }
}


template <bool NOVA>
__device__ __forceinline__ void fill_store(uint32_t e, uint32_t w0, uint32_t w1, uint32_t par, bool in, uint8_t *p) {
  const uint32_t f = (e >> 10) & 31u;
  const bool word = (e & 0x8000u) != 0;
  uint4 v;
  v.x = par ? 0u : (word ? w0 : (w0 >> f) & 1u);
  v.y = (!par && word && (f & 1u)) ? w1 : 0u;
  v.z = 0; v.w = 0;
  if (in) store16<false>(p, v);
}
template <bool ZONE>
__device__ __forceinline__ void fill_store_nova(uint32_t e, uint32_t w0, uint32_t w1, uint32_t par, bool ok, __amdgpu_buffer_rsrc_t rsrc, uint32_t rel,
                                                uint32_t body, uint32_t lane) {
  const uint32_t f = (e >> 10) & 31u;
  const bool word = (e & 0x8000u) != 0;
  u32x4 v;
  v.x = par ? 0u : (word ? w0 : (w0 >> f) & 1u);
  v.y = (!par && word && (f & 1u)) ? w1 : 0u;
  v.z = 0; v.w = 0;
  bool skip = false;
  if (ZONE) {
    const uint64_t wide = __builtin_amdgcn_ballot_w64(word && f == 2u && rel < body);
    skip = ((uint32_t)(wide >> (lane & 56u)) & 0xFFu) != 0;
  }
  const uint32_t off = (ok && !skip) ? rel : 0xFFFFFFF0u;
  __builtin_amdgcn_raw_buffer_store_b128(v, rsrc, (int)off, 0, 0);
}

#define B3W_LDS_STWORD 46
template <bool NOVA>
__device__ __forceinline__ void fill_report(const uint32_t *img, uint32_t w, uint32_t lane, uint32_t *__restrict__ pub, int32_t *__restrict__ status) {
  if (!NOVA) {
    if (pub && lane < 16) pub[(uint64_t)w * 16 + lane] = img[B3W_A_O + lane];
    if (status && lane == 16) status[w] = 0;
    return;
  }
  if (pub && lane < 15 && img[B3W_LDS_OKWORD]) {
    const uint32_t *nv = img + B3W_LDS_NV;
    const uint32_t src = lane == 0 ? B3W_LDS_NV + NV_N_BLOCKS : lane == 1 ? B3W_LDS_NV + NV_BLOCK_COUNT_OUT : lane < 10 ? B3W_A_O + (lane - 2)
                       : lane == 10 ? B3W_LDS_NV + NV_TOTAL_DEPTH : lane == 11 ? B3W_LDS_NV + NV_DEPTH_OUT : lane == 12 ? B3W_LDS_NV + NV_CIL
                       : lane == 13 ? B3W_LDS_NV + NV_CIH : B3W_LDS_NV + NV_LEAF_DEPTH;
    (void)nv;
    pub[(uint64_t)w * 15 + lane] = img[src];
  }
  if (status && lane == 16) status[w] = (int32_t)img[B3W_LDS_STWORD];
}

template <int NH, int NREC>
struct TracerRecs { uint32_t r[(NH * NREC + 63) / 64]; };
template <int NH, int NREC, typename WOf>
__device__ __forceinline__ void tracer_load(TracerRecs<NH, NREC> &t, const uint32_t *__restrict__ recs, uint32_t cnt, uint32_t lane, WOf w_of) {
#pragma unroll
  for (int c = 0; c < (NH * NREC + 63) / 64; ++c) {
    const uint32_t i = lane + 64u * c, k = i / NREC, j = i - k * NREC;
    t.r[c] = k < cnt ? recs[(uint64_t)w_of(k) * NREC + j] : 0u;
  }
}
template <int NH, int NREC, int WORDS, int DST>
__device__ __forceinline__ void tracer_put(const TracerRecs<NH, NREC> &t, uint32_t *half, uint32_t cnt, uint32_t lane) {
#pragma unroll
  for (int c = 0; c < (NH * NREC + 63) / 64; ++c) {
    const uint32_t i = lane + 64u * c, k = i / NREC, j = i - k * NREC;
    if (k < cnt) half[k * WORDS + DST + j] = t.r[c];
  }
  __builtin_amdgcn_fence(__ATOMIC_RELEASE, "wavefront");
  __builtin_amdgcn_wave_barrier();
}

#define B3W_RF_RING 256
struct RegionList {
  uint32_t n, body32, pitch32, off0, end;
  uint32_t grp, v_next, produced;
  int32_t zlo, zhi, xoff;
  bool done;
};
#define B3W_RF_STARTS 0x80000000u
#define B3W_RF_NEAR 0x40000000u
#define B3W_RF_REJECT 0x20000000u
#define B3W_RF_BODY 0x1FFFFFFFu
__device__ __forceinline__ void region_list_batch(RegionList &s, uint2 *ring, uint32_t lane) {
  const uint32_t v = s.v_next + lane, j = s.grp + 32u * v;
  const bool valid = (uint64_t)j << 12 < s.end;
  const uint32_t rs = j << 12, re = rs + 4096u;
  const uint32_t w_lo = (valid && rs >= s.off0 + s.body32) ? (rs - s.off0 - s.body32) / s.pitch32 + 1u : 0u;
  const uint32_t bs = s.off0 + w_lo * s.pitch32;
  const bool e1 = valid && w_lo < s.n && bs < re;
  const bool e2 = e1 && w_lo + 1 < s.n && bs + s.pitch32 < re;
  const uint64_t b1 = __builtin_amdgcn_ballot_w64(e1), b2 = __builtin_amdgcn_ballot_w64(e2), lt = (1ull << lane) - 1;
  const uint32_t pos = s.produced + __builtin_popcountll(b1 & lt) + __builtin_popcountll(b2 & lt);
  auto near = [&](int32_t rel) { const int32_t t = rel + s.xoff; return (t + 96 + 3072 + 35 > s.zlo && t < s.zhi + 4) ? B3W_RF_NEAR : 0u; };
  if (e1) ring[pos % B3W_RF_RING] = make_uint2(w_lo | (bs >= rs ? B3W_RF_STARTS : 0u) | near((int32_t)(rs - bs)), (uint32_t)((int32_t)(rs - bs) << 5));
  if (e2) ring[(pos + 1) % B3W_RF_RING] = make_uint2((w_lo + 1) | B3W_RF_STARTS | near((int32_t)(rs - bs - s.pitch32)), (uint32_t)((int32_t)(rs - bs - s.pitch32) << 5));
  s.produced = uni(s.produced + (uint32_t)__builtin_popcountll(b1) + (uint32_t)__builtin_popcountll(b2));
  s.v_next += 64;
  s.done = s.done || __builtin_amdgcn_ballot_w64(!valid) != 0;
}

template <int KIND, int NH>
__global__ __launch_bounds__(320, 1) void b3w_regionfill_kernel(const uint32_t *__restrict__ recs, uint32_t n,
                                                                uint8_t *__restrict__ out, uint64_t pitch,
                                                                const uint32_t *__restrict__ table, uint32_t nwit,
                                                                uint32_t *__restrict__ pub, int32_t *__restrict__ status, uint32_t pace,
                                                                const uint32_t *__restrict__ aux) {
  constexpr bool NOVA = KIND != B3W_KIND_COMP;
  constexpr int WORDS = NOVA ? B3W_LDS_WIDE : B3W_LDS_WORDS_COMP, NREC = NOVA ? 32 : 28, RDST = NOVA ? B3W_LDS_NV : B3W_A_H, R = 4;
  extern __shared__ __attribute__((aligned(16))) uint32_t bf_lds[];
  __shared__ uint2 ring[B3W_RF_RING];
  __shared__ uint32_t cnt_ring[4];
  uint16_t *tab = reinterpret_cast<uint16_t *>(bf_lds);
  const uint32_t tabw = ((nwit + 7u) & ~7u) / 2;
  uint32_t *lds = bf_lds + tabw;
  const uint32_t wave = uni(threadIdx.x >> 6), lane = threadIdx.x & 63u;
  const uint32_t x = blockIdx.x & 7u, grp = blockIdx.x >> 3;
  const uint32_t body = 32u * nwit;
  if (wave < 4) {
    const uint32_t padded = ((nwit + 31u) / 32u + 8u) * 32u;
    const uint4 *t8 = reinterpret_cast<const uint4 *>(table + padded);
    uint4 *tab8 = reinterpret_cast<uint4 *>(tab);
    const uint32_t n8 = (nwit + 7u) / 8u;
    for (uint32_t base8 = 0; base8 < n8; base8 += 256u * 4u) {
      uint4 v[4];
#pragma unroll
      for (int uu = 0; uu < 4; ++uu) {
        const uint32_t i8 = base8 + 256u * uu + threadIdx.x;
        v[uu] = i8 < n8 ? t8[i8] : make_uint4(0, 0, 0, 0);
      }
#pragma unroll
      for (int uu = 0; uu < 4; ++uu) {
        const uint32_t i8 = base8 + 256u * uu + threadIdx.x;
        if (i8 < n8) tab8[i8] = v[uu];
      }
    }
  }
  if (wave == 4) {
    const uint32_t q = lane >> 2, col = lane & 3;
    RegionList rl;
    rl.n = n; rl.body32 = nwit; rl.pitch32 = (uint32_t)(pitch >> 5);
    rl.off0 = (uint32_t)((reinterpret_cast<uint64_t>(out) & ((1ull << 17) - 1)) >> 5);
    rl.end = rl.off0 + (n - 1) * rl.pitch32 + rl.body32;
    rl.grp = grp; rl.v_next = 0; rl.produced = 0; rl.done = false;
    rl.xoff = (int32_t)(x << 7);
    rl.zlo = NOVA ? (int32_t)aux[B3W_AUX_WIDE_SLOTS] : 0x7FFFFFFF;
    rl.zhi = NOVA ? (int32_t)aux[B3W_AUX_WIDE_SLOTS + B3W_NOVA_ISZERO - 1] : -1;
    auto list_until = [&](uint32_t target) {
      while (!rl.done && rl.produced < target) region_list_batch(rl, ring, lane);
      __builtin_amdgcn_fence(__ATOMIC_RELEASE, "wavefront");
      __builtin_amdgcn_wave_barrier();
    };
    auto cnt_of = [&](uint32_t h) { return rl.produced <= h * NH ? 0u : (rl.produced - h * NH < (uint32_t)NH ? rl.produced - h * NH : (uint32_t)NH); };
    uint32_t al[3] = {0, 0, 0};
    if (NOVA) {
      const uint32_t na = aux[B3W_AUX_ALIAS_COUNT];
#pragma unroll
      for (int u = 0; u < 3; ++u) al[u] = lane + 64u * u < na ? aux[B3W_AUX_ALIAS_LIST + lane + 64u * u] : 0u;
    }
    TracerRecs<NH, NREC> tr;
    list_until(2 * NH);
    tracer_load<NH, NREC>(tr, recs, cnt_of(0), lane, [&](uint32_t k) { return ring[k % B3W_RF_RING].x & B3W_RF_BODY; });
    for (uint32_t h = 0;; ++h) {
      uint32_t *half = lds + (h & 1) * NH * WORDS;
      list_until((h + 3) * NH);
      const uint32_t cnt = cnt_of(h);
      if (lane == 0) cnt_ring[h & 3] = cnt;
      tracer_put<NH, NREC, WORDS, RDST>(tr, half, cnt, lane);
      tracer_load<NH, NREC>(tr, recs, cnt_of(h + 1), lane, [&](uint32_t k) { return ring[((h + 1) * NH + k) % B3W_RF_RING].x & B3W_RF_BODY; });
      if (!NOVA) {
        if (q < cnt) trace_compression(half + q * WORDS, col, nullptr);
      } else {
        if (q < cnt) {
          uint32_t *L = half + q * WORDS;
          const bool dom_a = nova_iszero_flags_quad(L, (int)col);
          const int32_t st = nova_select(L, (int)col, dom_a);
          if (col == 0) {
            L[B3W_LDS_OKWORD] = st == 0 ? 1u : 0u; L[B3W_LDS_STWORD] = (uint32_t)st;
            if (st != 0) ring[(h * NH + q) % B3W_RF_RING].x |= B3W_RF_REJECT;
          }
          if (st == 0) trace_compression(L, col, nullptr);
        }
        __builtin_amdgcn_fence(__ATOMIC_RELEASE, "wavefront");
        __builtin_amdgcn_wave_barrier();
        {
        uint32_t av[NH * 3];
#pragma unroll
        for (int qq = 0; qq < NH; ++qq)
#pragma unroll
          for (int u = 0; u < 3; ++u) av[qq * 3 + u] = ((uint32_t)qq < cnt && al[u]) ? half[qq * WORDS + (al[u] & 0xFFFFu)] : 0u;
#pragma unroll
        for (int qq = 0; qq < NH; ++qq)
#pragma unroll
          for (int u = 0; u < 3; ++u) if ((uint32_t)qq < cnt && al[u]) half[qq * WORDS + (al[u] >> 16)] = av[qq * 3 + u];
        }
      }
      __syncthreads();
      if (cnt < (uint32_t)NH) break;
    }
    return;
  }
  __builtin_amdgcn_s_setprio(3);
  const uint32_t par = lane & 1u;
  const uint32_t sub = wave;
  struct Ent { uint32_t wq; int32_t rel0, relw; uint32_t e[R]; };
  struct Wd { uint32_t w0[R], w1[R]; };
  auto s1 = [&](uint32_t k, Ent &en) {
    const uint2 d = ring[k % B3W_RF_RING];
    en.wq = uni(d.x);
    en.relw = (int32_t)uni(d.y) + (int32_t)((x << 12) + (sub << 10));
    en.rel0 = en.relw + (int32_t)(lane << 4);
    const int32_t s0 = en.rel0 >> 5;
    const uint16_t *tp = tab + s0;
#pragma unroll
    for (int r = 0; r < R; ++r) en.e[r] = tp[1024 * r];
  };
  auto s2 = [&](const Ent &en, Wd &wd, const uint32_t *img) {
#pragma unroll
    for (int r = 0; r < R; ++r) {
      const uint32_t *L = img + (en.e[r] & 0x3FFu);
      wd.w0[r] = L[0]; wd.w1[r] = L[1];
    }
  };
  auto s3 = [&](const Ent &en, const Wd &wd, const uint32_t *img) {
    if (NOVA || !(en.wq & B3W_RF_STARTS)) {
      for (uint32_t z = 0; z < (pace & 15u); ++z) __builtin_amdgcn_s_sleep(1);
      uint32_t pv = lane;
      for (uint32_t z = 0; z < (pace >> 4); ++z) asm volatile("v_add_u32 %0, %0, 1" : "+v"(pv));
    }
    const uint32_t w = en.wq & B3W_RF_BODY;
    if ((en.wq >> 31) && x == 0 && sub == 0) fill_report<NOVA>(img, w, lane, pub, status);
    uint8_t *dst = out + (uint64_t)w * pitch;
    if (NOVA) {
      const bool ok = !(en.wq & B3W_RF_REJECT);
      const __amdgpu_buffer_rsrc_t rsrc = __builtin_amdgcn_make_buffer_rsrc(dst, 0, (int)body, 0x00020000);
      if (en.wq & B3W_RF_NEAR) {
#pragma unroll
        for (int r = 0; r < R; ++r) fill_store_nova<true>(en.e[r], wd.w0[r], wd.w1[r], par, ok, rsrc, (uint32_t)(en.rel0 + (int32_t)(r << 15)), body, lane);
      } else {
#pragma unroll
        for (int r = 0; r < R; ++r) fill_store_nova<false>(en.e[r], wd.w0[r], wd.w1[r], par, ok, rsrc, (uint32_t)(en.rel0 + (int32_t)(r << 15)), body, lane);
      }
    } else {
#pragma unroll
      for (int r = 0; r < R; ++r) {
        const uint32_t rel = (uint32_t)(en.rel0 + (int32_t)(r << 15));
        fill_store<NOVA>(en.e[r], wd.w0[r], wd.w1[r], par, rel < body, dst + rel);
      }
    }
  };
  for (uint32_t h = 0;; ++h) {
    __syncthreads();
    const uint32_t cnt = uni(cnt_ring[h & 3]);
    const uint32_t *half = lds + (h & 1) * NH * WORDS;
    const uint32_t k0 = h * NH;
    Ent e0, e1, e2;
    Wd d0, d1, d2;
    if (0 < cnt) s1(k0, e0);
    if (1 < cnt) s1(k0 + 1, e1);
    if (0 < cnt) s2(e0, d0, half);
    for (uint32_t i = 0; i < cnt; i += 3) {
      if (i + 2 < cnt) s1(k0 + i + 2, e2);
      if (i + 1 < cnt) s2(e1, d1, half + (i + 1) * WORDS);
      s3(e0, d0, half + i * WORDS);
      if (i + 1 >= cnt) break;
      if (i + 3 < cnt) s1(k0 + i + 3, e0);
      if (i + 2 < cnt) s2(e2, d2, half + (i + 2) * WORDS);
      s3(e1, d1, half + (i + 1) * WORDS);
      if (i + 2 >= cnt) break;
      if (i + 4 < cnt) s1(k0 + i + 4, e1);
      if (i + 3 < cnt) s2(e0, d0, half + (i + 3) * WORDS);
      s3(e2, d2, half + (i + 2) * WORDS);
    }
    if (cnt < (uint32_t)NH) break;
  }
}

}

namespace {
template <bool WIDE, int K>
int launch_sweep(const uint32_t *d_images, uint32_t n, uint8_t *d_out, uint64_t pitch, const uint32_t *d_table,
                 uint32_t nwit, hipStream_t stream) {
  const uintptr_t addr = reinterpret_cast<uintptr_t>(d_out);
  if (pitch >= (1ull << 30) || (addr & 31)) return -5;
  const uint32_t lead = (uint32_t)(addr & 4095);
  static const int shape = getenv("B3W_SWEEP_SHAPE") ? atoi(getenv("B3W_SWEEP_SHAPE")) : 2;
  const size_t smem = (size_t)nwit * 4 + 16;
  constexpr size_t B3W_SWEEP_MAX_SMEM = 24614 * 4 + 16;
  if (smem > B3W_SWEEP_MAX_SMEM) return -5;
#define B3W_SWEEP_LAUNCH(PAIRS, SPLIT)                                                                              \
  {                                                                                                                 \
             \
    static std::atomic<uint64_t> attr_done{0};                                                                      \
    int dev = 0;                                                                                                    \
    (void)hipGetDevice(&dev);                                                                                       \
    const uint64_t bit = 1ull << (dev & 63);                                                                        \
    if (!(attr_done.load(std::memory_order_acquire) & bit)) {                                                       \
      hipError_t e = hipFuncSetAttribute(reinterpret_cast<const void *>(&b3w_sweep_kernel<WIDE, K, B3W_SWEEP_LOGC, PAIRS, SPLIT>), \
                                         hipFuncAttributeMaxDynamicSharedMemorySize, (int)B3W_SWEEP_MAX_SMEM);     \
      if (e != hipSuccess) return (int)e;                                                                           \
      attr_done.fetch_or(bit, std::memory_order_release);                                                           \
    }                                                                                                               \
    hipLaunchKernelGGL((b3w_sweep_kernel<WIDE, K, B3W_SWEEP_LOGC, PAIRS, SPLIT>), dim3(B3W_SWEEP_GRID), dim3(128 * PAIRS), smem, \
                       stream, d_images, n, d_out - lead, lead, (uint32_t)pitch, d_table, nwit);                    \
  }
  switch (shape) {
    case 1: B3W_SWEEP_LAUNCH(1, false); break;
    case 3: B3W_SWEEP_LAUNCH(4, true); break;
    case 4: B3W_SWEEP_LAUNCH(3, true); break;
    case 0: B3W_SWEEP_LAUNCH(2, false); break;
    default: B3W_SWEEP_LAUNCH(2, true); break;
  }
#undef B3W_SWEEP_LAUNCH
  return (int)hipGetLastError();
}
}

extern "C" int b3w_launch_verify(int kind, const uint32_t *d_in_slots, uint32_t n, const uint8_t *d_bodies, uint64_t pitch,
                                 const uint32_t *d_table, uint32_t nwit, uint32_t *d_mismatch, const void *d_aux,
                                 hipStream_t stream) {
  if (n == 0) return 0;
  uint8_t *bodies = const_cast<uint8_t *>(d_bodies);
  const uint32_t pm = (uint32_t)(pitch >> 5) & 3u, stride = (pitch & 31) ? 1u : pm == 0 ? 1u : pm == 2 ? 2u : 4u;
#define B3W_VGRID(WV) dim3((n + stride * WV - 1) / (stride * WV) * stride)
  if (kind == B3W_KIND_COMP)
    hipLaunchKernelGGL((b3w_compression_kernel<4, false, 2>), B3W_VGRID(4), dim3(64), 0, stream, d_in_slots, n, bodies, pitch,
                       d_table, nwit, d_mismatch, (int32_t *)nullptr, stride);
  else if (kind == B3W_KIND_NOVA_O2)
    hipLaunchKernelGGL((b3w_nova_kernel<B3W_KIND_NOVA_O2, 2, false, 2>), B3W_VGRID(2), dim3(64), 0, stream, d_in_slots, n,
                       bodies, pitch, d_table, nwit, d_mismatch, (int32_t *)nullptr, (const uint32_t *)d_aux, stride);
  else
    hipLaunchKernelGGL((b3w_nova_kernel<B3W_KIND_NOVA_O1, 2, false, 2>), B3W_VGRID(2), dim3(64), 0, stream, d_in_slots, n,
                       bodies, pitch, d_table, nwit, d_mismatch, (int32_t *)nullptr, (const uint32_t *)d_aux, stride);
#undef B3W_VGRID
  return (int)hipGetLastError();
}

extern "C" int b3w_launch_trace(int kind, const uint32_t *d_recs, uint32_t cn, uint32_t *d_images, uint32_t row, const uint32_t *d_table,
                                uint32_t nwit, uint32_t *d_pub, int32_t *d_status, const void *d_aux, hipStream_t stream) {
  if (cn == 0) return 0;
  if (cn > row) return -4;
  if (kind == B3W_KIND_COMP)
    hipLaunchKernelGGL((b3w_compression_kernel<16, false, 1>), dim3((cn + 15) / 16), dim3(64), 0, stream, d_recs, cn,
                       reinterpret_cast<uint8_t *>(d_images), (uint64_t)row, d_table, nwit, d_pub, d_status, 1u);
  else if (kind == B3W_KIND_NOVA_O2)
    hipLaunchKernelGGL((b3w_nova_kernel<B3W_KIND_NOVA_O2, 4, false, 1>), dim3((cn + 3) / 4), dim3(64), 0, stream, d_recs, cn,
                       reinterpret_cast<uint8_t *>(d_images), (uint64_t)row, d_table, nwit, d_pub, d_status, (const uint32_t *)d_aux, 1u);
  else if (kind == B3W_KIND_NOVA_O1)
    hipLaunchKernelGGL((b3w_nova_kernel<B3W_KIND_NOVA_O1, 2, false, 1>), dim3((cn + 1) / 2), dim3(64), 0, stream, d_recs, cn,
                       reinterpret_cast<uint8_t *>(d_images), (uint64_t)row, d_table, nwit, d_pub, d_status, (const uint32_t *)d_aux, 1u);
  else return -2;
  return (int)hipGetLastError();
}

extern "C" int b3w_launch_batch(int kind, int variant, const uint32_t *d_recs, uint32_t n, uint8_t *d_out,
                                uint64_t pitch, const uint32_t *d_table, uint32_t nwit, uint32_t *d_pub,
                                int32_t *d_status, const void *d_aux, uint32_t *d_scratch, uint32_t scratch_cap,
                                hipStream_t stream) {
  if (n == 0) return 0;
  if (variant >= B3W_VARIANT_SWEEP && variant < B3W_VARIANT_REGIONFILL) {
    if (!d_scratch || scratch_cap != (1u << B3W_SWEEP_LOGC)) return -4;
    if (kind != B3W_KIND_COMP && !d_aux) return -3;
    uint32_t *d_images = d_scratch;
    for (uint32_t c0 = 0; c0 < n; c0 += scratch_cap) {
      const uint32_t cn = n - c0 < scratch_cap ? n - c0 : scratch_cap;
      uint32_t *pub_c = d_pub ? d_pub + (uint64_t)c0 * (kind == B3W_KIND_COMP ? 16 : 15) : nullptr;
      int32_t *st_c = d_status ? d_status + c0 : nullptr;
      uint8_t *out_c = d_out + (uint64_t)c0 * pitch;
      int rc = b3w_launch_trace(kind, d_recs + (uint64_t)c0 * (kind == B3W_KIND_COMP ? 28 : 32), cn, d_images, scratch_cap, d_table, nwit, pub_c,
                                st_c, d_aux, stream);
      if (rc) return rc;
      if (kind == B3W_KIND_COMP) rc = launch_sweep<false, 8>(d_images, cn, out_c, pitch, d_table, nwit, stream);
      else rc = launch_sweep<true, 4>(d_images, cn, out_c, pitch, d_table, nwit, stream);
      if (rc) return rc;
    }
    return (int)hipGetLastError();
  }
  if (variant == B3W_VARIANT_REGIONFILL || variant == B3W_VARIANT_REGIONFILL_LIGHT) {
    if (kind != B3W_KIND_COMP && kind != B3W_KIND_NOVA_O2) return -1;
    if (kind == B3W_KIND_NOVA_O2 && !d_aux) return -3;
    if ((reinterpret_cast<uintptr_t>(d_out) & 31) || (pitch & 31) || pitch >= (1ull << 30)) return -5;
    if (32ull * nwit < (1ull << 17) || (uint64_t)n * pitch + (1ull << 20) >= (1ull << 37)) return -5;
    constexpr int NH_C = 14, NH_N = 11;
    const bool nova = kind != B3W_KIND_COMP;
    const size_t smem = (size_t)((nwit + 7u) & ~7u) * 2 +
                        (size_t)(2 * (nova ? NH_N * B3W_LDS_WIDE : NH_C * B3W_LDS_WORDS_COMP) + 4) * 4;
    constexpr size_t B3W_FILL_MAX_SMEM = 160 * 1024 - 4096;
    if (smem > B3W_FILL_MAX_SMEM) return -5;
    static std::atomic<uint64_t> attr_done{0};
    int dev = 0;
    (void)hipGetDevice(&dev);
    const uint64_t bit = 1ull << (dev & 63);
    if (!(attr_done.load(std::memory_order_acquire) & bit)) {
      hipError_t e = hipFuncSetAttribute(reinterpret_cast<const void *>(&b3w_regionfill_kernel<B3W_KIND_COMP, NH_C>),
                                         hipFuncAttributeMaxDynamicSharedMemorySize, (int)B3W_FILL_MAX_SMEM);
      if (e == hipSuccess)
        e = hipFuncSetAttribute(reinterpret_cast<const void *>(&b3w_regionfill_kernel<B3W_KIND_NOVA_O2, NH_N>), hipFuncAttributeMaxDynamicSharedMemorySize,
                                (int)B3W_FILL_MAX_SMEM);
      if (e != hipSuccess) return (int)e;
      attr_done.fetch_or(bit, std::memory_order_release);
    }
    const char *pace_s = getenv("B3W_FILL_PACE");
    const int pace_env = pace_s ? atoi(pace_s) : -1;
    const uint32_t pace = pace_env >= 0 ? (uint32_t)pace_env : variant == B3W_VARIANT_REGIONFILL_LIGHT ? (nova ? 33u : 48u) : nova ? 18u : 33u;
    if (!nova) {
      hipLaunchKernelGGL((b3w_regionfill_kernel<B3W_KIND_COMP, NH_C>), dim3(B3W_REGIONFILL_GRID), dim3(320), smem, stream, d_recs, n, d_out, pitch,
                         d_table, nwit, d_pub, d_status, pace, (const uint32_t *)nullptr);
    } else {
      hipLaunchKernelGGL((b3w_regionfill_kernel<B3W_KIND_NOVA_O2, NH_N>), dim3(B3W_REGIONFILL_GRID), dim3(320), smem, stream, d_recs, n, d_out, pitch,
                         d_table, nwit, d_pub, d_status, pace, (const uint32_t *)d_aux);
      hipLaunchKernelGGL((b3w_nova_kernel<B3W_KIND_NOVA_O2, 2, false, 3>), dim3((n + 1) / 2), dim3(64), 0, stream, d_recs, n, d_out, pitch, d_table, nwit,
                         (uint32_t *)nullptr, (int32_t *)nullptr, (const uint32_t *)d_aux, 1u);
    }
    return (int)hipGetLastError();
  }
  if (variant > B3W_VARIANT_REGIONFILL_LIGHT) return -1;
  const uint32_t pm = (uint32_t)(pitch >> 5) & 3u, stride = (pitch & 31) ? 1u : pm == 0 ? 1u : pm == 2 ? 2u : 4u;
#define B3W_GRID(WV) dim3((n + stride * WV - 1) / (stride * WV) * stride)
  static const uint32_t lds_pad = getenv("B3W_LDS_PAD") ? (uint32_t)atoi(getenv("B3W_LDS_PAD")) : 0;
  if (kind == B3W_KIND_COMP) {
#define B3W_LAUNCH_COMP(WV, NTV)                                                                         \
  hipLaunchKernelGGL((b3w_compression_kernel<WV, NTV, 0>), B3W_GRID(WV), dim3(64), lds_pad, stream,        \
                     d_recs, n, d_out, pitch, d_table, nwit, d_pub, d_status, stride)
    if (variant >= B3W_VARIANT_SLICED && variant < B3W_VARIANT_SWEEP) {
      const uint32_t slices = (uint32_t)(variant - B3W_VARIANT_SLICED);
      if (slices < 2 || slices > 64) return -1;
      hipLaunchKernelGGL((b3w_compression_kernel<1, false, 0, true>), dim3(B3W_GRID(1).x * slices), dim3(64), 0, stream, d_recs, n, d_out,
                         pitch, d_table, nwit, d_pub, d_status, stride, slices);
      return (int)hipGetLastError();
    }
    switch (variant) {
      case 0: B3W_LAUNCH_COMP(4, false); break;
      case 1: B3W_LAUNCH_COMP(1, false); break;
      case 2: B3W_LAUNCH_COMP(2, false); break;
      case 3: B3W_LAUNCH_COMP(8, false); break;
      case 4: B3W_LAUNCH_COMP(4, true); break;
      case 5: B3W_LAUNCH_COMP(2, true); break;
      case 6: B3W_LAUNCH_COMP(1, true); break;
      case 7: B3W_LAUNCH_COMP(16, false); break;
      case 8:
        hipLaunchKernelGGL((b3w_compression_kernel<8, false, 0>), B3W_GRID(8), dim3(64), lds_pad ? lds_pad : 24576u, stream, d_recs, n, d_out,
                           pitch, d_table, nwit, d_pub, d_status, stride);
        break;
      default: return -1;
    }
#undef B3W_LAUNCH_COMP
    return (int)hipGetLastError();
  }
  if (kind == B3W_KIND_NOVA_O2 || kind == B3W_KIND_NOVA_O1) {
    if (!d_aux) return -3;
#define B3W_LAUNCH_NOVA(KV, WV)                                                                           \
  hipLaunchKernelGGL((b3w_nova_kernel<KV, WV, false, 0>), B3W_GRID(WV), dim3(64), lds_pad, stream,          \
                     d_recs, n, d_out, pitch, d_table, nwit, d_pub, d_status, (const uint32_t *)d_aux, stride)
#define B3W_LAUNCH_NOVA_P(KV, WV, G)                                                                            \
  hipLaunchKernelGGL((b3w_nova_kernel<KV, WV, false, 0, false, true>), dim3(B3W_GRID(WV).x < (G) ? B3W_GRID(WV).x : (G)), dim3(64), lds_pad, stream, \
                     d_recs, n, d_out, pitch, d_table, nwit, d_pub, d_status, (const uint32_t *)d_aux, stride)
    if (variant >= B3W_VARIANT_SLICED && variant < B3W_VARIANT_SWEEP) {
      const uint32_t slices = (uint32_t)(variant - B3W_VARIANT_SLICED);
      if (slices < 2 || slices > 64) return -1;
      if (kind == B3W_KIND_NOVA_O2)
        hipLaunchKernelGGL((b3w_nova_kernel<B3W_KIND_NOVA_O2, 1, false, 0, true>), dim3(B3W_GRID(1).x * slices), dim3(64), 0, stream, d_recs, n,
                           d_out, pitch, d_table, nwit, d_pub, d_status, (const uint32_t *)d_aux, stride, slices);
      else
        hipLaunchKernelGGL((b3w_nova_kernel<B3W_KIND_NOVA_O1, 1, false, 0, true>), dim3(B3W_GRID(1).x * slices), dim3(64), 0, stream, d_recs, n,
                           d_out, pitch, d_table, nwit, d_pub, d_status, (const uint32_t *)d_aux, stride, slices);
      return (int)hipGetLastError();
    }
    if (kind == B3W_KIND_NOVA_O2) {
      switch (variant) {
        case 0: B3W_LAUNCH_NOVA(B3W_KIND_NOVA_O2, 2); break;
        case 1: B3W_LAUNCH_NOVA(B3W_KIND_NOVA_O2, 1); break;
        case 2: B3W_LAUNCH_NOVA(B3W_KIND_NOVA_O2, 4); break;
        case 3: B3W_LAUNCH_NOVA(B3W_KIND_NOVA_O2, 8); break;
        case 4: B3W_LAUNCH_NOVA_P(B3W_KIND_NOVA_O2, 8, 512u); break;
        default: return -1;
      }
    } else {
      switch (variant) {
        case 0: B3W_LAUNCH_NOVA(B3W_KIND_NOVA_O1, 2); break;
        case 1: B3W_LAUNCH_NOVA(B3W_KIND_NOVA_O1, 1); break;
        default: return -1;
      }
    }
#undef B3W_LAUNCH_NOVA
#undef B3W_LAUNCH_NOVA_P
    return (int)hipGetLastError();
  }
  return -2;
}
```

Measured before the change: 9.357 million.

## Interleave BLAKE3 trace rounds with witness expansion stores in compression kernel

Adds a host-side table of phase boundaries that records, per output alignment shift, which witness tiles depend only on words produced by earlier trace rounds. The compression kernel (MODE 0) now runs the seven trace rounds incrementally and emits those output tiles as soon as their inputs are ready, so global stores overlap the round computation instead of waiting for the full trace. It also adds dealt multi-workgroup variants (2 or 4 slices, with LDS padding sized for four workgroups per CU) to the autotune candidates, plus optional wall-clock stamps for debugging. The cost is more intricate control flow, extra wave-level fences per round, and a risk of wrong ordering if the phase table misjudges dependencies.

```diff
diff --git a/hot-proofs-blake3-circom_amd/build.py b/hot-proofs-blake3-circom_amd/build.py
--- a/hot-proofs-blake3-circom_amd/build.py
+++ b/hot-proofs-blake3-circom_amd/build.py
@@ -37,7 +37,7 @@
     objdir = os.path.join(PKG, "build")
     os.makedirs(objdir, exist_ok=True)
     if os.environ.get("B3W_BUILD_DIAG") == "1":
-        extra_flags = (*extra_flags, "-DB3W_R1CS_DIAG")
+        extra_flags = (*extra_flags, "-DB3W_R1CS_DIAG", "-DB3W_STREAM_STAMPS")
     flags = [f"--offload-arch={ARCH}", "-O3", "-std=c++17", "-fPIC", "-x", "hip", "-Wall", "-Wno-unused-function", *extra_flags]
     jobs = []
     for src in srcs:
diff --git a/hot-proofs-blake3-circom_amd/csrc/b3w_ctx.cpp b/hot-proofs-blake3-circom_amd/csrc/b3w_ctx.cpp
--- a/hot-proofs-blake3-circom_amd/csrc/b3w_ctx.cpp
+++ b/hot-proofs-blake3-circom_amd/csrc/b3w_ctx.cpp
@@ -249,6 +249,39 @@
 
 bool b3w_int_build_slot_table(const CircuitDesc &c, std::vector<uint32_t> &table, std::string &err) { return build_slot_table(c, table, err); }
 
+void b3w_int_stream_phases(const CircuitDesc &c, uint32_t j, uint32_t out[9]) {
+  const uint32_t jlo = j < 4 ? j : 0, jhi = j < 4 ? j : 3;
+  const uint32_t ntiles = (c.nwit + jlo + 31) / 32;
+  for (int i = 0; i < 9; i++) out[i] = 0;
+  out[8] = ntiles;
+  std::vector<uint32_t> table;
+  std::string err;
+  if (c.kind != B3W_KIND_COMP || !build_slot_table(c, table, err)) return;
+  auto word_round = [](uint32_t w) -> int { return w >= B3W_A_H && w < B3W_A_O ? -1 : w >= B3W_LDS_HG && w < B3W_LDS_WORDS_COMP ? (int)((w - B3W_LDS_HG) / 128) : 7; };
+  std::vector<int> ready(ntiles, -1);
+  for (uint32_t k = 0; k < ntiles; k++) {
+    for (int64_t s = 32ll * k - jhi; s < 32ll * k - jlo + 32; s++) {
+      if (s < 0 || s >= (int64_t)c.nwit) continue;
+      const uint32_t e = table[s], src = e & 0xFFFu, mode = (e >> 17) & 3u;
+      for (uint32_t i = 0; i < (mode == B3W_MODE_W256 ? 8u : mode == B3W_MODE_W64 ? 2u : 1u); i++) ready[k] = std::max(ready[k], word_round(src + i));
+    }
+  }
+  uint32_t k0 = 0;
+  while (k0 < ntiles && ready[k0] != 0) k0++;
+  if (k0 == ntiles) return;
+  uint32_t b[7];
+  int run = -1;
+  uint32_t r = 0;
+  for (uint32_t pos = 0; pos < ntiles - k0; pos++) {
+    run = std::max(run, ready[k0 + pos]);
+    for (; r < 7 && (int)r < run; r++) b[r] = pos & ~3u;
+  }
+  for (; r < 7; r++) b[r] = (ntiles - k0) & ~3u;
+  if (2 * b[6] < ntiles) return;
+  out[0] = k0;
+  for (r = 0; r < 7; r++) out[1 + r] = b[r];
+}
+
 namespace {
 int32_t ensure_scratch(b3w_ctx *ctx) {
   if (ctx->d_scratch) return B3W_OK;
@@ -288,6 +321,12 @@
 extern "C" {
 
 uint32_t b3w_abi_version(void) { return (1u << 16) | 4u; }
+
+int32_t b3w_stream_phases(int32_t circuit, uint32_t j, uint32_t out[9]) {
+  if (circuit < 0 || circuit > 3 || j >= B3W_STREAM_SHIFTS || !out) return B3W_E_BAD_ARGUMENT;
+  b3w_int_stream_phases(CIRCUITS[circuit], j, out);
+  return B3W_OK;
+}
 
 int32_t b3w_identify_wasm(const uint8_t *code, size_t len) {
   if (!code) return B3W_CIRCUIT_UNKNOWN;
@@ -372,6 +411,11 @@
       if (mode == B3W_MODE_W64 && src + 1 >= 1024) { ctx->fill_ok = false; continue; }
       ftab[i] = (uint16_t)(mode == B3W_MODE_BIT ? (src | sh << 10) : (src | (mode == B3W_MODE_W64 ? 1u : 0u) << 10 | 0x8000u));
     }
+  }
+  for (uint32_t j = 0; j < B3W_STREAM_SHIFTS; j++) {
+    uint32_t t[9];
+    b3w_int_stream_phases(ctx->desc, j, t);
+    memcpy(&ctx->phases[j], t, sizeof t);
   }
   DeviceGuard guard(device);
   if (guard.err != hipSuccess) { delete ctx; return B3W_E_NO_DEVICE; }
@@ -519,7 +563,7 @@
   if (ctx->variant_auto || (ctx->variant_tuned && n <= 2560)) variant = b3w_int_default_variant(ctx, n, d_bodies, pitch);
   if (variant >= B3W_VARIANT_REGIONFILL && !ctx->fill_ok) { ctx->last_error = "the fill-ordered variants (200, 201) exist for the compression circuit and the nova O2 builds"; return B3W_E_BAD_ARGUMENT; }
   int rc = b3w_launch_batch(ctx->desc.kind, variant, d_records, n, d_bodies, pitch, ctx->d_table, ctx->desc.nwit,
-                            d_public, d_status, ctx->d_aux, ctx->d_scratch, ctx->scratch_cap, (hipStream_t)stream);
+                            d_public, d_status, ctx->d_aux, ctx->d_scratch, ctx->scratch_cap, ctx->phases, (hipStream_t)stream);
   if (rc == 0) return B3W_OK;
   if (rc == -5) { ctx->last_error = "the sweep and fill-ordered paths need 32-byte aligned bodies and pitch < 2^30"; return B3W_E_BAD_ARGUMENT; }
   if (rc < 0) { ctx->last_error = "no kernel for this circuit kind / variant"; return B3W_E_BAD_ARGUMENT; }
@@ -560,17 +604,20 @@
   }
   rc = ensure_scratch(ctx);
   if (rc) return rc;
-  const int candidates[6] = {0, ctx->desc.kind == B3W_KIND_COMP ? (n > 6144 ? 8 : 3) : ctx->desc.kind == B3W_KIND_NOVA_O2 ? 3 : 0, B3W_VARIANT_SWEEP,
-                             ctx->fill_ok ? B3W_VARIANT_REGIONFILL : 0, ctx->desc.kind == B3W_KIND_NOVA_O2 && n >= 16384 ? 4 : 0,
-                             ctx->fill_ok ? B3W_VARIANT_REGIONFILL_LIGHT : 0};
+  constexpr int NCAND = 8;
+  const bool comp = ctx->desc.kind == B3W_KIND_COMP;
+  const int candidates[NCAND] = {0, comp ? (n > 6144 ? 8 : 3) : ctx->desc.kind == B3W_KIND_NOVA_O2 ? 3 : 0, B3W_VARIANT_SWEEP,
+                                 ctx->fill_ok ? B3W_VARIANT_REGIONFILL : 0, ctx->desc.kind == B3W_KIND_NOVA_O2 && n >= 16384 ? 4 : 0,
+                                 ctx->fill_ok ? B3W_VARIANT_REGIONFILL_LIGHT : 0, comp ? B3W_VARIANT_DEALT2 : 0, comp ? B3W_VARIANT_DEALT4 : 0};
   int best = ctx->variant;
   float best_ms = 1e30f;
   const int saved = ctx->variant;
   const bool saved_auto = ctx->variant_auto;
   ctx->variant_auto = false;
-  float cand_ms[6] = {1e30f, 1e30f, 1e30f, 1e30f, 1e30f, 1e30f};
+  float cand_ms[NCAND];
+  for (float &v : cand_ms) v = 1e30f;
   for (int round = 0; round < 2; round++) {
-    for (int ci = 0; ci < 6; ci++) {
+    for (int ci = 0; ci < NCAND; ci++) {
       const int c = candidates[ci];
       if (ci > 0 && c == candidates[0]) continue;
       if (round > 0 && cand_ms[ci] >= 1e30f) continue;
@@ -585,7 +632,7 @@
       if (ms < cand_ms[ci]) cand_ms[ci] = ms;
     }
   }
-  for (int ci = 0; ci < 6; ci++)
+  for (int ci = 0; ci < NCAND; ci++)
     if (cand_ms[ci] < best_ms) { best_ms = cand_ms[ci]; best = candidates[ci]; }
   if (best_ms >= 1e30f) { ctx->variant = saved; ctx->variant_auto = saved_auto; return B3W_E_BAD_ARGUMENT; }
   ctx->variant = best;
diff --git a/hot-proofs-blake3-circom_amd/csrc/b3w_internal.h b/hot-proofs-blake3-circom_amd/csrc/b3w_internal.h
--- a/hot-proofs-blake3-circom_amd/csrc/b3w_internal.h
+++ b/hot-proofs-blake3-circom_amd/csrc/b3w_internal.h
@@ -60,6 +60,7 @@
   uint32_t *d_fe_inputs = nullptr;
   uint32_t *d_status2 = nullptr;
   uint32_t *d_in_slots = nullptr;
+  B3wStreamPhases phases[B3W_STREAM_SHIFTS]{};
   uint32_t scratch_cap = 0;
   uint32_t *d_rec1 = nullptr;
   uint8_t *d_body1 = nullptr;
@@ -134,6 +135,9 @@
   if (_dev_guard.err != hipSuccess) return hip_fail(ctx, _dev_guard.err, "hipSetDevice")
 
 bool b3w_int_build_slot_table(const CircuitDesc &c, std::vector<uint32_t> &table, std::string &err);
+void b3w_int_stream_phases(const CircuitDesc &c, uint32_t j, uint32_t out[9]);
+extern "C" int32_t b3w_stream_phases(int32_t circuit, uint32_t j, uint32_t out[9]);
+static_assert(sizeof(B3wStreamPhases) == 9 * sizeof(uint32_t), "b3w_int_stream_phases fills a B3wStreamPhases");
 int b3w_int_default_variant(const b3w_ctx *ctx, uint32_t n, const uint8_t *d_bodies, uint64_t pitch);
 b3w_ctx *b3w_int_key_ctx(const b3w_commit_key *key);
 int32_t b3w_int_commit_records(b3w_ctx *ctx, const b3w_commit_key *key, const uint32_t *d_records, uint32_t n, uint8_t *d_points, uint32_t *d_public,
diff --git a/hot-proofs-blake3-circom_amd/csrc/b3w_kernels.h b/hot-proofs-blake3-circom_amd/csrc/b3w_kernels.h
--- a/hot-proofs-blake3-circom_amd/csrc/b3w_kernels.h
+++ b/hot-proofs-blake3-circom_amd/csrc/b3w_kernels.h
@@ -18,10 +18,18 @@
 #define B3W_SWEEP_LOGC 13
 #define B3W_SWEEP_CHUNK (1u << B3W_SWEEP_LOGC)
 
+#define B3W_VARIANT_DEALT2 92
+#define B3W_VARIANT_DEALT4 94
+struct B3wStreamPhases { uint32_t k0, b[8]; };
+#define B3W_STREAM_SHIFTS 5
+
 extern "C" int b3w_launch_batch(int kind, int variant, const uint32_t *d_recs, uint32_t n, uint8_t *d_out,
                                 uint64_t pitch, const uint32_t *d_table, uint32_t nwit, uint32_t *d_pub,
                                 int32_t *d_status, const void *d_aux, uint32_t *d_scratch, uint32_t scratch_cap,
-                                hipStream_t stream);
+                                const B3wStreamPhases *phases , hipStream_t stream);
+#ifdef B3W_STREAM_STAMPS
+extern "C" int b3w_dbg_stream_stamps(unsigned long long *d_stamps, uint32_t workgroups);
+#endif
 
 extern "C" int b3w_launch_exact(int nova, const uint32_t *d_inputs, const uint32_t *d_prime, const uint32_t *d_table,
                                 uint32_t nwit, uint8_t *d_out, uint32_t *d_status, hipStream_t stream);
diff --git a/hot-proofs-blake3-circom_amd/csrc/b3w_kernels.hip b/hot-proofs-blake3-circom_amd/csrc/b3w_kernels.hip
--- a/hot-proofs-blake3-circom_amd/csrc/b3w_kernels.hip
+++ b/hot-proofs-blake3-circom_amd/csrc/b3w_kernels.hip
@@ -8,6 +8,23 @@
 namespace {
 
 typedef uint32_t u32x4 __attribute__((ext_vector_type(4)));
+
+__device__ __forceinline__ void wave_lds_fence() {
+  __builtin_amdgcn_fence(__ATOMIC_RELEASE, "wavefront");
+  __builtin_amdgcn_wave_barrier();
+  __builtin_amdgcn_fence(__ATOMIC_ACQUIRE, "wavefront");
+}
+
+#ifdef B3W_STREAM_STAMPS
+__device__ unsigned long long *b3w_stamps = nullptr;
+__device__ uint32_t b3w_stamps_cap = 0;
+#define B3W_STAMP(i)                                                                                            \
+  do {                                                                                                          \
+    if (b3w_stamps && threadIdx.x == 0 && blockIdx.x < b3w_stamps_cap) b3w_stamps[blockIdx.x * 4 + (i)] = wall_clock64(); \
+  } while (0)
+#else
+#define B3W_STAMP(i) do {} while (0)
+#endif
 
 __device__ __forceinline__ uint32_t rotr32(uint32_t x, int r) { return __builtin_rotateright32(x, r); }
 
@@ -68,24 +85,44 @@
   d = quad_perm<1, 2, 3, 0>(d);
 }
 
-__device__ __forceinline__ void trace_compression(uint32_t *L, int col, uint32_t *pub ) {
+struct TraceState { uint32_t a, b, c, d, h_lo, h_hi; };
+__device__ __forceinline__ TraceState trace_begin(const uint32_t *L, int col) {
   const uint32_t IVc = col == 0 ? 0x6A09E667u : col == 1 ? 0xBB67AE85u : col == 2 ? 0x3C6EF372u : 0xA54FF53Au;
-  uint32_t a = L[B3W_A_H + col], b = L[B3W_A_H + 4 + col], c = IVc, d = L[B3W_A_T + col];
-  const uint32_t h_lo = a, h_hi = b;
-  round_fn<0>(a, b, c, d, L, L, col);
-  round_fn<1>(a, b, c, d, L, L, col);
-  round_fn<2>(a, b, c, d, L, L, col);
-  round_fn<3>(a, b, c, d, L, L, col);
-  round_fn<4>(a, b, c, d, L, L, col);
-  round_fn<5>(a, b, c, d, L, L, col);
-  round_fn<6>(a, b, c, d, L, L, col);
-  const uint32_t o0 = a ^ c, o1 = b ^ d, o2 = c ^ h_lo, o3 = d ^ h_hi;
+  const uint32_t a = L[B3W_A_H + col], b = L[B3W_A_H + 4 + col], d = L[B3W_A_T + col];
+  return TraceState{a, b, IVc, d, a, b};
+}
+template <int R>
+__device__ __forceinline__ void trace_round(TraceState &t, uint32_t *L, int col) { round_fn<R>(t.a, t.b, t.c, t.d, L, L, col); }
+__device__ __forceinline__ void trace_round(TraceState &t, uint32_t *L, int col, int r) {
+  switch (r) {
+    case 0: trace_round<0>(t, L, col); break;
+    case 1: trace_round<1>(t, L, col); break;
+    case 2: trace_round<2>(t, L, col); break;
+    case 3: trace_round<3>(t, L, col); break;
+    case 4: trace_round<4>(t, L, col); break;
+    case 5: trace_round<5>(t, L, col); break;
+    default: trace_round<6>(t, L, col); break;
+  }
+}
+__device__ __forceinline__ void trace_finish(const TraceState &t, uint32_t *L, int col, uint32_t *pub ) {
+  const uint32_t o0 = t.a ^ t.c, o1 = t.b ^ t.d, o2 = t.c ^ t.h_lo, o3 = t.d ^ t.h_hi;
   L[B3W_A_O + col] = o0;
   L[B3W_A_O + 4 + col] = o1;
   L[B3W_A_O + 8 + col] = o2;
   L[B3W_A_O + 12 + col] = o3;
   if (col == 0) L[B3W_A_ONE] = 1u;
   if (pub) { pub[col] = o0; pub[4 + col] = o1; pub[8 + col] = o2; pub[12 + col] = o3; }
+}
+__device__ __forceinline__ void trace_compression(uint32_t *L, int col, uint32_t *pub ) {
+  TraceState t = trace_begin(L, col);
+  trace_round<0>(t, L, col);
+  trace_round<1>(t, L, col);
+  trace_round<2>(t, L, col);
+  trace_round<3>(t, L, col);
+  trace_round<4>(t, L, col);
+  trace_round<5>(t, L, col);
+  trace_round<6>(t, L, col);
+  trace_finish(t, L, col, pub);
 }
 
 template <bool NT>
@@ -136,55 +173,87 @@
 }
 
 template <int W, int WORDS, bool WIDE, bool NT>
+struct Expand {
+  static constexpr int U = 4;
+  const uint32_t *lds, *tp, *okmask;
+  uint8_t *out;
+  uint32_t nwit, nact, j, ntiles, kf0, kf1;
+  bool fast;
+  int lane;
+  uint64_t woff[W];
+#ifdef B3W_STREAM_STAMPS
+  mutable bool stamped = false;
+  __device__ __forceinline__ void first_store() const { if (!stamped) { stamped = true; B3W_STAMP(2); } }
+#else
+  __device__ __forceinline__ void first_store() const {}
+#endif
+  __device__ __forceinline__ Expand(const uint32_t *lds_, const uint32_t *__restrict__ table, uint32_t nwit_, uint8_t *__restrict__ out_,
+                                    uint64_t pitch, const WaveBodies wb, uint32_t n, const uint32_t *okmask_ ,
+                                    bool all_ok)
+      : lds(lds_), okmask(okmask_), out(out_), nwit(nwit_), lane(threadIdx.x) {
+    nact = wave_active<W>(wb, n);
+    const uint64_t start = reinterpret_cast<uint64_t>(out) + (uint64_t)wb.first * pitch;
+    j = (start & 31) ? 0u : (uint32_t)(start >> 5) & 3u;
+    ntiles = (nwit + j + 31) >> 5;
+    kf0 = j ? 1u : 0u;
+    kf1 = (nwit + j) >> 5;
+    fast = nact == (uint32_t)W && all_ok;
+#pragma unroll
+    for (int w = 0; w < W; ++w) woff[w] = (uint64_t)wb(w) * pitch + (uint32_t)lane * 16u - 32u * j;
+    tp = table + (lane >> 1) - j;
+  }
+  __device__ __forceinline__ void tiles(uint32_t k, uint32_t kend) const { tiles(k, kend, [](uint32_t) __attribute__((always_inline)) {}); }
+  template <class Before>
+  __device__ __forceinline__ void tiles(uint32_t k, uint32_t kend, Before &&before) const {
+    uint64_t wo[W];
+#pragma unroll
+    for (int w = 0; w < W; ++w) wo[w] = woff[w] + (uint64_t)k * 1024u;
+    auto ragged = [&](uint32_t ke) __attribute__((always_inline)) {
+      for (; k < ke; ++k) {
+        const uint32_t slot = k * 32 + (lane >> 1) - j;
+        before(k);
+        emit_group<W, WORDS, WIDE, NT, false>(lds, tp[k * 32], out, wo, 0, slot < nwit, nact, okmask);
+        first_store();
+#pragma unroll
+        for (int w = 0; w < W; ++w) wo[w] += 1024u;
+      }
+    };
+    if (fast) {
+      ragged(kf0 < kend ? kf0 : kend);
+      const uint32_t kf1s = kf1 < kend ? kf1 : kend;
+      uint32_t cur[U], nxt[U];
+#pragma unroll
+      for (int u = 0; u < U; ++u) cur[u] = tp[(k + u) * 32];
+      for (; k + U <= kf1s; k += U) {
+#pragma unroll
+        for (int u = 0; u < U; ++u) nxt[u] = tp[(k + U + u) * 32];
+        before(k + U - 1);
+#pragma unroll
+        for (int u = 0; u < U; ++u) emit_group<W, WORDS, WIDE, NT, true>(lds, cur[u], out, wo, u * 1024u, true, nact, nullptr);
+        first_store();
+#pragma unroll
+        for (int w = 0; w < W; ++w) wo[w] += U * 1024u;
+#pragma unroll
+        for (int u = 0; u < U; ++u) cur[u] = nxt[u];
+      }
+    }
+    ragged(kend);
+  }
+  __device__ __forceinline__ void part(uint32_t lo, uint32_t hi, uint32_t slice, uint32_t slices) const {
+    const uint32_t per = ((hi - lo + slices - 1) / slices + (U - 1)) & ~(uint32_t)(U - 1);
+    const uint32_t k = lo + slice * per < hi ? lo + slice * per : hi;
+    tiles(k, k + per < hi ? k + per : hi);
+  }
+};
+
+template <int W, int WORDS, bool WIDE, bool NT>
 __device__ __forceinline__ void expand(const uint32_t *lds, const uint32_t *__restrict__ table, uint32_t nwit,
                                        uint8_t *__restrict__ out, uint64_t pitch, const WaveBodies wb, uint32_t n,
                                        const uint32_t *okmask , bool all_ok,
                                        uint32_t slice = 0, uint32_t slices = 1 ) {
-  constexpr int U = 4;
-  const int lane = threadIdx.x;
-  const uint32_t nact = wave_active<W>(wb, n);
-  const uint64_t start = reinterpret_cast<uint64_t>(out) + (uint64_t)wb.first * pitch;
-  const uint32_t j = (start & 31) ? 0u : (uint32_t)(start >> 5) & 3u;
-  const uint32_t ntiles = (nwit + j + 31) >> 5;
-  const uint32_t kf0 = j ? 1u : 0u, kf1 = (nwit + j) >> 5;
-  uint64_t woff[W];
-#pragma unroll
-  for (int w = 0; w < W; ++w) woff[w] = (uint64_t)wb(w) * pitch + (uint32_t)lane * 16u - 32u * j;
-  const uint32_t *tp = table + (lane >> 1) - j;
-  uint32_t k = 0, kend_all = ntiles;
-  if (slices > 1) {
-    const uint32_t per = ((ntiles + slices - 1) / slices + (U - 1)) & ~(uint32_t)(U - 1);
-    k = slice * per < ntiles ? slice * per : ntiles;
-    kend_all = k + per < ntiles ? k + per : ntiles;
-#pragma unroll
-    for (int w = 0; w < W; ++w) woff[w] += (uint64_t)k * 1024u;
-  }
-  const uint32_t kf1s = kf1 < kend_all ? kf1 : kend_all;
-  auto ragged = [&](uint32_t kend) {
-    for (; k < kend; ++k) {
-      const uint32_t slot = k * 32 + (lane >> 1) - j;
-      emit_group<W, WORDS, WIDE, NT, false>(lds, tp[k * 32], out, woff, 0, slot < nwit, nact, okmask);
-#pragma unroll
-      for (int w = 0; w < W; ++w) woff[w] += 1024u;
-    }
-  };
-  if (nact == (uint32_t)W && all_ok) {
-    ragged(kf0 < kend_all ? kf0 : kend_all);
-    uint32_t cur[U], nxt[U];
-#pragma unroll
-    for (int u = 0; u < U; ++u) cur[u] = tp[(k + u) * 32];
-    for (; k + U <= kf1s; k += U) {
-#pragma unroll
-      for (int u = 0; u < U; ++u) nxt[u] = tp[(k + U + u) * 32];
-#pragma unroll
-      for (int u = 0; u < U; ++u) emit_group<W, WORDS, WIDE, NT, true>(lds, cur[u], out, woff, u * 1024u, true, nact, nullptr);
-#pragma unroll
-      for (int w = 0; w < W; ++w) woff[w] += U * 1024u;
-#pragma unroll
-      for (int u = 0; u < U; ++u) cur[u] = nxt[u];
-    }
-  }
-  ragged(kend_all);
+  const Expand<W, WORDS, WIDE, NT> ex(lds, table, nwit, out, pitch, wb, n, okmask, all_ok);
+  if (slices > 1) ex.part(0, ex.ntiles, slice, slices);
+  else ex.tiles(0, ex.ntiles);
 }
 
 template <int W, int WORDS, bool WIDE>
@@ -415,14 +484,17 @@
                                                              uint8_t *__restrict__ out, uint64_t pitch,
                                                              const uint32_t *__restrict__ table, uint32_t nwit,
                                                              uint32_t *__restrict__ pub, int32_t *__restrict__ status,
-                                                             uint32_t stride , uint32_t slices = 1) {
+                                                             uint32_t stride , uint32_t slices = 1,
+                                                             B3wStreamPhases ph = B3wStreamPhases{}) {
   constexpr int WORDS = B3W_LDS_WORDS_COMP;
   __shared__ __attribute__((aligned(16))) uint32_t lds[W * WORDS + 4];
   const int lane = threadIdx.x;
-  const uint32_t slice = SL ? blockIdx.x % slices : 0u;
+  const uint32_t groups = SL && W > 1 ? gridDim.x / slices : 1u;
+  const uint32_t slice = !SL ? 0u : W > 1 ? blockIdx.x / groups : blockIdx.x % slices;
   if (SL && slice != 0) { pub = nullptr; status = nullptr; }
+  B3W_STAMP(0);
  for (uint32_t bid = blockIdx.x;; bid += gridDim.x) {
-  const WaveBodies wb = wave_bodies<W>(SL ? bid / slices : bid, stride);
+  const WaveBodies wb = wave_bodies<W>(!SL ? bid : W > 1 ? bid % groups : bid / slices, stride);
   if (wb.first >= n) return;
   const uint32_t wit0 = wb.first;
   __shared__ uint32_t ncf[W];
@@ -443,6 +515,55 @@
     }
   }
   __syncthreads();
+  B3W_STAMP(1);
+  if (MODE == 0) {
+    const int w = lane >> 2, col = lane & 3;
+    const bool tracer = w < W && wb(w) < n;
+    uint32_t *L = lds + (tracer ? w : 0) * WORDS;
+    const Expand<W, WORDS, false, NT> ex(lds, table, nwit, out, pitch, wb, n, nullptr, true);
+    const uint32_t k0 = ph.k0 < ex.ntiles ? ph.k0 : ex.ntiles, asc = ex.ntiles - k0;
+    TraceState t{};
+    if (tracer) t = trace_begin(L, col);
+    int done = 0;
+    auto reach = [&](uint32_t pos) __attribute__((always_inline)) {
+      while (done < 7 && (done == 0 || pos >= (ph.b[done - 1] < asc ? ph.b[done - 1] : asc))) {
+        if (tracer) {
+          trace_round(t, L, col, done);
+          if (done == 6) {
+            trace_finish(t, L, col, pub ? pub + (uint64_t)wb(w) * 16 : nullptr);
+            if (status && col == 0) status[wb(w)] = 0;
+          }
+        }
+        ++done;
+        wave_lds_fence();
+      }
+    };
+    if (SL && W > 1) {
+      uint32_t lo = 0;
+#pragma unroll 1
+      for (int r = 0; r < 7; ++r) {
+        const uint32_t b = ph.b[r] < asc ? ph.b[r] : asc, hi = b > lo ? b : lo;
+        if (hi > lo) { reach(lo); ex.part(k0 + lo, k0 + hi, slice, slices); }
+        lo = hi;
+      }
+      reach(~0u);
+      ex.part(k0 + lo, ex.ntiles, slice, slices);
+      ex.part(0, k0, slice, slices);
+    } else {
+      const uint32_t per = ((ex.ntiles + slices - 1) / slices + 3u) & ~3u;
+      const uint32_t own0 = !SL ? 0u : slice * per < ex.ntiles ? slice * per : ex.ntiles;
+      const uint32_t own1 = !SL ? ex.ntiles : own0 + per < ex.ntiles ? own0 + per : ex.ntiles;
+      if (own1 > k0) ex.tiles(own0 > k0 ? own0 : k0, own1, [&](uint32_t k) __attribute__((always_inline)) { reach(k - k0); });
+      if (!SL || slice == 0 || own0 < k0) {
+        reach(~0u);
+        ex.tiles(own0, own1 < k0 ? own1 : k0);
+      }
+    }
+    B3W_STAMP(3);
+    if (!PERSIST) return;
+    __syncthreads();
+    continue;
+  }
   {
     const int w = lane >> 2, col = lane & 3;
     if (w < W && wb(w) < n) {
@@ -452,12 +573,11 @@
   }
   __syncthreads();
   if (MODE == 1) dump_images<W, WORDS>(lds, reinterpret_cast<uint32_t *>(out), (uint32_t)pitch, wit0, n, nullptr);
-  else if (MODE == 2) {
+  else {
     uint32_t cnt[W];
     expand_verify<W, WORDS, false>(lds, table, nwit, out, pitch, wb, n, cnt);
     publish_counts<W>(cnt, pub, wb, n, ncf);
-  } else if (SL) expand<W, WORDS, false, NT>(lds, table, nwit, out, pitch, wb, n, nullptr, true, slice, slices);
-  else expand<W, WORDS, false, NT>(lds, table, nwit, out, pitch, wb, n, nullptr, true);
+  }
   if (!PERSIST) return;
   __syncthreads();
  }
@@ -1145,10 +1265,18 @@
   return (int)hipGetLastError();
 }
 
+#ifdef B3W_STREAM_STAMPS
+extern "C" int b3w_dbg_stream_stamps(unsigned long long *d_stamps, uint32_t workgroups) {
+  hipError_t e = hipMemcpyToSymbol(HIP_SYMBOL(b3w_stamps_cap), &workgroups, sizeof workgroups);
+  if (e == hipSuccess) e = hipMemcpyToSymbol(HIP_SYMBOL(b3w_stamps), &d_stamps, sizeof d_stamps);
+  return (int)e;
+}
+#endif
+
 extern "C" int b3w_launch_batch(int kind, int variant, const uint32_t *d_recs, uint32_t n, uint8_t *d_out,
                                 uint64_t pitch, const uint32_t *d_table, uint32_t nwit, uint32_t *d_pub,
                                 int32_t *d_status, const void *d_aux, uint32_t *d_scratch, uint32_t scratch_cap,
-                                hipStream_t stream) {
+                                const B3wStreamPhases *phases, hipStream_t stream) {
   if (n == 0) return 0;
   if (variant >= B3W_VARIANT_SWEEP && variant < B3W_VARIANT_REGIONFILL) {
     if (!d_scratch || scratch_cap != (1u << B3W_SWEEP_LOGC)) return -4;
@@ -1211,14 +1339,25 @@
 #define B3W_GRID(WV) dim3((n + stride * WV - 1) / (stride * WV) * stride)
   static const uint32_t lds_pad = getenv("B3W_LDS_PAD") ? (uint32_t)atoi(getenv("B3W_LDS_PAD")) : 0;
   if (kind == B3W_KIND_COMP) {
+    static const bool staged = !(getenv("B3W_STREAM_PHASES") && atoi(getenv("B3W_STREAM_PHASES")) == 0);
+    const uintptr_t addr = reinterpret_cast<uintptr_t>(d_out);
+    const B3wStreamPhases ph = !(phases && staged) ? B3wStreamPhases{} : phases[(addr & 31) ? 0u : stride == 1 ? (uint32_t)(addr >> 5) & 3u : 4u];
 #define B3W_LAUNCH_COMP(WV, NTV)                                                                         \
   hipLaunchKernelGGL((b3w_compression_kernel<WV, NTV, 0>), B3W_GRID(WV), dim3(64), lds_pad, stream,        \
-                     d_recs, n, d_out, pitch, d_table, nwit, d_pub, d_status, stride)
+                     d_recs, n, d_out, pitch, d_table, nwit, d_pub, d_status, stride, 1u, ph)
+    if (variant == B3W_VARIANT_DEALT2 || variant == B3W_VARIANT_DEALT4) {
+      const uint32_t slices = variant == B3W_VARIANT_DEALT2 ? 2u : 4u;
+      constexpr uint32_t image = (4 * B3W_LDS_WORDS_COMP + 4 + 4) * 4, pad = 36u * 1024u - image;
+      static_assert(image < 32u * 1024u && image + pad > 32u * 1024u && image + pad <= 40u * 1024u, "the request admits four workgroups per CU");
+      hipLaunchKernelGGL((b3w_compression_kernel<4, false, 0, true>), dim3(B3W_GRID(4).x * slices), dim3(64), pad, stream, d_recs, n, d_out,
+                         pitch, d_table, nwit, d_pub, d_status, stride, slices, ph);
+      return (int)hipGetLastError();
+    }
     if (variant >= B3W_VARIANT_SLICED && variant < B3W_VARIANT_SWEEP) {
       const uint32_t slices = (uint32_t)(variant - B3W_VARIANT_SLICED);
       if (slices < 2 || slices > 64) return -1;
       hipLaunchKernelGGL((b3w_compression_kernel<1, false, 0, true>), dim3(B3W_GRID(1).x * slices), dim3(64), 0, stream, d_recs, n, d_out,
-                         pitch, d_table, nwit, d_pub, d_status, stride, slices);
+                         pitch, d_table, nwit, d_pub, d_status, stride, slices, ph);
       return (int)hipGetLastError();
     }
     switch (variant) {
@@ -1232,7 +1371,7 @@
       case 7: B3W_LAUNCH_COMP(16, false); break;
       case 8:
         hipLaunchKernelGGL((b3w_compression_kernel<8, false, 0>), B3W_GRID(8), dim3(64), lds_pad ? lds_pad : 24576u, stream, d_recs, n, d_out,
-                           pitch, d_table, nwit, d_pub, d_status, stride);
+                           pitch, d_table, nwit, d_pub, d_status, stride, 1u, ph);
         break;
       default: return -1;
     }
```

Result: no change. 9.370 million, median of 4 (+0.1%).
